# biotite-dev/springcraft

Hardware: AMD Instinct MI355X
Metric: ANM modes/sec (Hessian build + full eigensolve), N=2000 C-alpha (higher is better)
Workload: dtype f64; 1 GPU; C3: N=2000 C-alpha ANM, HinsenForceField (no cutoff), full 6000x6000 eigensolve, all modes + vectors; parallelism=independent structures sharded over GPUs, no data-path collective

## Files before the change

### include/springcraft_hip_debug.h

```cpp
#ifndef SPRINGCRAFT_HIP_DEBUG_H
#define SPRINGCRAFT_HIP_DEBUG_H

#include "springcraft_hip.h"

#ifdef __cplusplus
extern "C" {
#endif

int sc_dbg_gemm_bench(sc_ctx* ctx, int m, int n, int k, int mode, int tile, int split_k, int iters, int beta_one,
                      double* ms_out, double* max_err_out);

int sc_dbg_gemm_host(sc_ctx* ctx, const double* a, const double* b, double* c, int m, int n, int k, int mode, int tile,
                     int split_k, double alpha, double beta, int lower_grid);

int sc_dbg_gemm3_host(sc_ctx* ctx, const double* a, const double* b, double* c, int count, int m, int n, int k, int layout,
                      int lower, double beta);

int sc_dbg_symm3_host(sc_ctx* ctx, const double* a, const double* v, double* x, int count, int m, int split);
int sc_dbg_symm3_stamps(unsigned long long* out4);
int sc_dbg_symm3_bench(sc_ctx* ctx, int count, int m, int split, int iters, double* ms_out);

int sc_dbg_gemm3_bench(sc_ctx* ctx, int count, int m, int n, int k, int layout, int lower, int kernel, int order, int iters,
                       double* ms_out);

int sc_dbg_gemm_stamps(unsigned long long* out4, int reset);

int sc_dbg_gemm_trace(unsigned long long* out, int max_records, int* count, int reset);

int sc_dbg_two_stage(sc_ctx* ctx, const double* a, int n, double* band_out, double* d_out, double* e_out);

int sc_dbg_bt2_stamps(unsigned long long* out);

int sc_dbg_bt2_clock(unsigned long long* out2);

int sc_dbg_bt2_trace(unsigned long long* out);

int sc_dbg_bulge_stamps(unsigned long long* out6);
int sc_dbg_pair_stamps(unsigned long long* out48);
int sc_dbg_chase_stamps(unsigned long long* out16);

int sc_dbg_set_chase(sc_ctx* ctx, int mode, int give_up_after);

int sc_dbg_set_panel_coop(sc_ctx* ctx, int min_rows);
int sc_dbg_set_panel_coop_fail(sc_ctx* ctx, int panel);

int sc_dbg_set_resident(sc_ctx* ctx, int mode, int hook, int workgroups);
int sc_dbg_resident_stamps(unsigned long long* out8);

#ifdef __cplusplus
}
#endif
#endif
```

### springcraft_amd/csrc/api.hip

```cpp
#include <algorithm>
#include <cmath>
#include <cstdarg>
#include <cstring>
#include <map>
#include <new>
#include <utility>

#include "common.h"
#include "host_logic.h"

int sc_set_error(sc_ctx* ctx, int code, const char* fmt, ...) {
  char buf[1024];
  va_list ap;
  va_start(ap, fmt);
  vsnprintf(buf, sizeof(buf), fmt, ap);
  va_end(ap);
  if (ctx) ctx->err = buf;
  return code;
}

static int reserve(sc_ctx* ctx, void*& buf, size_t& have, size_t bytes, bool collect_events = false) {
  if (bytes <= have) return SC_OK;
  if (buf) {
    SC_HIP(ctx, hipStreamSynchronize(ctx->stream));
// ... 98 lines not shown
  SC_HIP(ctx, hipStreamCreateWithFlags(&ctx->aux_stream, hipStreamNonBlocking));
  SC_HIP(ctx, hipEventCreateWithFlags(&ctx->aux_fork, hipEventDisableTiming));
  SC_HIP(ctx, hipEventCreateWithFlags(&ctx->aux_join, hipEventDisableTiming));
  return SC_OK;
}

int sc_side_streams(sc_ctx* ctx, int count) {
  while ((int)ctx->side_streams.size() < count) {
    hipStream_t s = nullptr;
    hipEvent_t e = nullptr;
    SC_HIP(ctx, hipStreamCreateWithFlags(&s, hipStreamNonBlocking));
    if (hipEventCreateWithFlags(&e, hipEventDisableTiming) != hipSuccess) {
      (void)hipStreamDestroy(s);
      return sc_set_error(ctx, SC_ERR_HIP, "hipEventCreateWithFlags failed");
    }
    ctx->side_streams.push_back(s);
    ctx->side_joins.push_back(e);
  }
  return SC_OK;
}

namespace {

int ctx_create_impl(int device, void* stream, bool own, sc_ctx** out) {
  if (!out) return SC_ERR_INVALID_ARG;
  *out = nullptr;
  int count = 0;
  if (hipGetDeviceCount(&count) != hipSuccess || count <= 0 || device < 0 || device >= count)
    return SC_ERR_NO_DEVICE;
  hipDeviceProp_t prop;
  if (hipGetDeviceProperties(&prop, device) != hipSuccess) return SC_ERR_NO_DEVICE;
  if (std::strncmp(prop.gcnArchName, "gfx950", 6) != 0) return SC_ERR_NO_DEVICE;
  if (hipSetDevice(device) != hipSuccess) return SC_ERR_NO_DEVICE;
  sc_ctx* ctx = new sc_ctx();
  ctx->device = device;
  ctx->num_cus = prop.multiProcessorCount;
  if (own) {
    if (hipStreamCreateWithFlags(&ctx->stream, hipStreamNonBlocking) != hipSuccess) {
      delete ctx;
      return SC_ERR_HIP;
    }
    ctx->own_stream = true;
  } else {
    ctx->stream = (hipStream_t)stream;
  }
  if (hipMalloc((void**)&ctx->d_status, kSpStatusWords * sizeof(unsigned long long)) != hipSuccess ||
      hipMemset(ctx->d_status, 0, kSpStatusWords * sizeof(unsigned long long)) != hipSuccess ||
      hipMalloc((void**)&ctx->d_zeros, 16384) != hipSuccess || hipMemset(ctx->d_zeros, 0, 16384) != hipSuccess ||
      hipMalloc((void**)&ctx->d_chase_ctl, kChaseCtlInts * sizeof(int)) != hipSuccess ||
      hipMemset(ctx->d_chase_ctl, 0, kChaseCtlInts * sizeof(int)) != hipSuccess ||
      hipDeviceSynchronize() != hipSuccess) {
    if (ctx->d_status) (void)hipFree(ctx->d_status);
    if (ctx->d_zeros) (void)hipFree(ctx->d_zeros);
    if (ctx->d_chase_ctl) (void)hipFree(ctx->d_chase_ctl);
    if (ctx->own_stream) (void)hipStreamDestroy(ctx->stream);
    delete ctx;
    return SC_ERR_NOMEM;
  }
  *out = ctx;
  return SC_OK;
}

int check_ff(sc_ctx* ctx, const sc_ff_desc* ff) {
  std::string err;
  const int rc = sc_host::check_ff(ff, err);
  return rc == SC_OK ? SC_OK : sc_set_error(ctx, rc, "%s", err.c_str());
}

struct Bump {
  char* base;
  size_t off = 0;
  template <typename T>
  T* take(size_t count) {
    off = align_up(off, 256);
    T* p = reinterpret_cast<T*>(base + off);
    off += count * sizeof(T);
    return p;
  }
};

using sc_host::HostPatch;

int build_patch(sc_ctx* ctx, const sc_patch_desc* pd, int64_t n, HostPatch& hp) {
  std::string err;
  const int rc = sc_host::build_patch(pd, n, hp, err);
  return rc == SC_OK ? SC_OK : sc_set_error(ctx, rc, "%s", err.c_str());
}

int upload_patch(sc_ctx* ctx, const HostPatch& hp, Bump& bump, PatchDev& dev) {
  uint8_t* d_shut = bump.take<uint8_t>(hp.shut.size());
  int32_t* d_rp = bump.take<int32_t>(hp.row_ptr.size());
  int32_t* d_col = bump.take<int32_t>(hp.col.size() + 1);
  int8_t* d_flag = bump.take<int8_t>(hp.flag.size() + 1);
  double* d_gam = bump.take<double>(hp.gam.size() + 1);
  SC_HIP(ctx, hipMemcpyAsync(d_shut, hp.shut.data(), hp.shut.size(), hipMemcpyHostToDevice, ctx->stream));
  SC_HIP(ctx, hipMemcpyAsync(d_rp, hp.row_ptr.data(), hp.row_ptr.size() * 4, hipMemcpyHostToDevice, ctx->stream));
  if (!hp.col.empty()) {
    SC_HIP(ctx, hipMemcpyAsync(d_col, hp.col.data(), hp.col.size() * 4, hipMemcpyHostToDevice, ctx->stream));
    SC_HIP(ctx, hipMemcpyAsync(d_flag, hp.flag.data(), hp.flag.size(), hipMemcpyHostToDevice, ctx->stream));
    SC_HIP(ctx, hipMemcpyAsync(d_gam, hp.gam.data(), hp.gam.size() * 8, hipMemcpyHostToDevice, ctx->stream));
  }
  SC_HIP(ctx, hipStreamSynchronize(ctx->stream));
  dev = PatchDev{d_shut, d_rp, d_col, d_flag, d_gam, hp.mask_gamma};
  return SC_OK;
}

int check_coord_args(sc_ctx* ctx, const double* coord, int64_t n) {
  if (!ctx) return SC_ERR_INVALID_ARG;
  if (n < 0 || n > 2000000) return sc_set_error(ctx, SC_ERR_INVALID_ARG, "bad atom count %lld", (long long)n);
  if (n > 0 && !coord) return sc_set_error(ctx, SC_ERR_INVALID_ARG, "coord is NULL");
  return SC_OK;
}

struct Staged {
  double* d_coord = nullptr;
  double* d_w = nullptr;
  PatchDev patch{};
  bool has_patch = false;
  HostPatch hp;
  sc_tab_desc tab_dev{};
  sc_ff_desc ff_dev{};
};

size_t tab_device_bytes(const sc_ff_desc* ff, int64_t n) {
  if (!ff || ff->kind != SC_FF_TABULATED || !ff->tab) return 0;
  const size_t nb = (size_t)ff->tab->n_bins;
  return align_up(nb * 8, 256) + align_up(3 * 400 * nb * 4, 256) + 2 * align_up((size_t)n * 4, 256) +
         align_up((size_t)n, 256) + 2048;
}

int stage_tab(sc_ctx* ctx, const sc_ff_desc* ff, int64_t n, Staged& st, Bump& bump) {
  st.ff_dev = *ff;
  if (ff->kind != SC_FF_TABULATED) return SC_OK;
  const sc_tab_desc* t = ff->tab;
  const size_t nb = (size_t)t->n_bins;
  for (int64_t i = 0; i < n; ++i)
    if (t->atom_type[i] < 0 || t->atom_type[i] >= 20)
      return sc_set_error(ctx, SC_ERR_INDEX, "amino-acid type %d of atom %lld out of range", t->atom_type[i],
                          (long long)i);
  double* d_edges = bump.take<double>(nb);
  float* d_tab = bump.take<float>(3 * 400 * nb);
  int32_t* d_type = bump.take<int32_t>((size_t)n);
  int32_t* d_chain = bump.take<int32_t>((size_t)n);
  uint8_t* d_bond = bump.take<uint8_t>((size_t)n);
  hipStream_t s = ctx->stream;
  if (t->edges_sq) SC_HIP(ctx, hipMemcpyAsync(d_edges, t->edges_sq, nb * 8, hipMemcpyHostToDevice, s));
  SC_HIP(ctx, hipMemcpyAsync(d_tab, t->bonded, 400 * nb * 4, hipMemcpyHostToDevice, s));
  SC_HIP(ctx, hipMemcpyAsync(d_tab + 400 * nb, t->intra_chain, 400 * nb * 4, hipMemcpyHostToDevice, s));
  SC_HIP(ctx, hipMemcpyAsync(d_tab + 800 * nb, t->inter_chain, 400 * nb * 4, hipMemcpyHostToDevice, s));
  SC_HIP(ctx, hipMemcpyAsync(d_type, t->atom_type, (size_t)n * 4, hipMemcpyHostToDevice, s));
  SC_HIP(ctx, hipMemcpyAsync(d_chain, t->chain, (size_t)n * 4, hipMemcpyHostToDevice, s));
  SC_HIP(ctx, hipMemcpyAsync(d_bond, t->bonded_next, (size_t)n, hipMemcpyHostToDevice, s));
  SC_HIP(ctx, hipStreamSynchronize(s));
  st.tab_dev = *t;
  st.tab_dev.edges_sq = d_edges;
  st.tab_dev.bonded = d_tab;
  st.tab_dev.intra_chain = d_tab + 400 * nb;
  st.tab_dev.inter_chain = d_tab + 800 * nb;
  st.tab_dev.atom_type = d_type;
  st.tab_dev.chain = d_chain;
  st.tab_dev.bonded_next = d_bond;
  st.ff_dev.tab = &st.tab_dev;
  return SC_OK;
}

int stage_inputs(sc_ctx* ctx, const double* coord, int64_t n, const sc_ff_desc* ff, const sc_patch_desc* pd,
                 const double* inv_sqrt_mass, size_t extra_bytes, Staged& st, Bump& bump) {
  SC_TRY(build_patch(ctx, pd, n, st.hp));
  size_t need = align_up((size_t)n * 24, 256) + align_up((size_t)n * 8, 256) + 1024 + extra_bytes +
                tab_device_bytes(ff, n);
  if (st.hp.any) need += st.hp.device_bytes();
  SC_TRY(sc_reserve_scratch(ctx, need));
  bump.base = (char*)ctx->scratch;
  bump.off = 0;
  st.d_coord = bump.take<double>((size_t)n * 3);
  SC_HIP(ctx, hipMemcpyAsync(st.d_coord, coord, (size_t)n * 24, hipMemcpyHostToDevice, ctx->stream));
  if (inv_sqrt_mass) {
    st.d_w = bump.take<double>((size_t)n);
    SC_HIP(ctx, hipMemcpyAsync(st.d_w, inv_sqrt_mass, (size_t)n * 8, hipMemcpyHostToDevice, ctx->stream));
  }
  if (st.hp.any) {
    SC_TRY(upload_patch(ctx, st.hp, bump, st.patch));
    st.has_patch = true;
  }
  SC_TRY(stage_tab(ctx, ff, n, st, bump));
  return SC_OK;
}

}

extern "C" {

int sc_ctx_create(int device, sc_ctx** out) { return ctx_create_impl(device, nullptr, true, out); }

int sc_ctx_create_on_stream(int device, void* hip_stream, sc_ctx** out) {
  return ctx_create_impl(device, hip_stream, false, out);
}

void sc_ctx_destroy(sc_ctx* ctx) {
  if (!ctx) return;
  (void)hipSetDevice(ctx->device);
  (void)hipStreamSynchronize(ctx->stream);
  if (ctx->ws) (void)hipFree(ctx->ws);
  if (ctx->scratch) (void)hipFree(ctx->scratch);
  if (ctx->dc_aux) (void)hipFree(ctx->dc_aux);
  if (ctx->pinv_ws) (void)hipFree(ctx->pinv_ws);
  if (ctx->win_ws) (void)hipFree(ctx->win_ws);
  if (ctx->modes_ws) (void)hipFree(ctx->modes_ws);
  if (ctx->d_status) (void)hipFree(ctx->d_status);
  if (ctx->d_zeros) (void)hipFree(ctx->d_zeros);
  if (ctx->d_chase_ctl) (void)hipFree(ctx->d_chase_ctl);
  for (int c = 0; c < 2; ++c) {
    if (ctx->h_stage[c]) (void)hipHostFree(ctx->h_stage[c]);
    if (ctx->h_stage_done[c]) (void)hipEventDestroy(ctx->h_stage_done[c]);
  }
  if (ctx->aux_stream) {
    (void)hipStreamSynchronize(ctx->aux_stream);
    (void)hipStreamDestroy(ctx->aux_stream);
    (void)hipEventDestroy(ctx->aux_fork);
    (void)hipEventDestroy(ctx->aux_join);
  }
  for (size_t i = 0; i < ctx->side_streams.size(); ++i) {
    (void)hipStreamSynchronize(ctx->side_streams[i]);
    (void)hipStreamDestroy(ctx->side_streams[i]);
    (void)hipEventDestroy(ctx->side_joins[i]);
  }
  if (ctx->own_stream) (void)hipStreamDestroy(ctx->stream);
  delete ctx;
}

const char* sc_last_error(sc_ctx* ctx) { return ctx ? ctx->err.c_str() : "null context"; }

int sc_host_alloc(size_t bytes, void** out) {
  if (!out || bytes == 0) return SC_ERR_INVALID_ARG;
  *out = nullptr;
  void* p = nullptr;
  if (hipHostMalloc(&p, bytes, hipHostMallocDefault) != hipSuccess || !p) {
    (void)hipGetLastError();
    return SC_ERR_NOMEM;
  }
  *out = p;
  return SC_OK;
}

int sc_host_free(void* p) {
  if (!p) return SC_OK;
  return hipHostFree(p) == hipSuccess ? SC_OK : SC_ERR_HIP;
}

int sc_ctx_synchronize(sc_ctx* ctx) {
  if (!ctx) return SC_ERR_INVALID_ARG;
  SC_HIP(ctx, hipSetDevice(ctx->device));
  SC_HIP(ctx, hipStreamSynchronize(ctx->stream));
  return sc_deferred_status(ctx);
}

int sc_device_info(sc_ctx* ctx, char* buf, size_t buflen) {
  if (!ctx || !buf || buflen == 0) return SC_ERR_INVALID_ARG;
  hipDeviceProp_t prop;
  SC_HIP(ctx, hipGetDeviceProperties(&prop, ctx->device));
  snprintf(buf, buflen, "%s %s, %d CUs, %.0f GiB", prop.gcnArchName, prop.name,
           prop.multiProcessorCount, (double)prop.totalGlobalMem / (1 << 30));
  return SC_OK;
}

int sc_ctx_set_profiling(sc_ctx* ctx, int enabled) {
  if (!ctx) return SC_ERR_INVALID_ARG;
  ctx->profiling = enabled != 0;
  return SC_OK;
}

int sc_last_eigh_timings(sc_ctx* ctx, double* out6) {
  if (!ctx || !out6) return SC_ERR_INVALID_ARG;
  for (int i = 0; i < 6; ++i) out6[i] = ctx->last_timings[i];
  return SC_OK;
}

int sc_last_eigh_phase_ms(sc_ctx* ctx, const char* name, double* ms) {
  if (!ctx || !name || !ms) return SC_ERR_INVALID_ARG;
  for (const auto& p : ctx->phases)
    if (p.first == name) { *ms = p.second; return SC_OK; }
  *ms = 0.0;
  return SC_ERR_INVALID_ARG;
}

int sc_ctx_get_counter(sc_ctx* ctx, const char* name, int64_t* value) {
  if (!ctx || !name || !value) return SC_ERR_INVALID_ARG;
  const std::string k(name);
  SC_HIP(ctx, hipSetDevice(ctx->device));
  SC_HIP(ctx, hipStreamSynchronize(ctx->stream));
  SC_TRY(sc_collect_events(ctx));
  int tmin = ctx->chase_tickets[0], tmax = ctx->chase_tickets[0];
  long long tsum = 0;
  for (int x = 0; x < std::max(1, std::min(8, ctx->chase_ctl_xcds)); ++x) {
    tmin = std::min(tmin, ctx->chase_tickets[x]);
    tmax = std::max(tmax, ctx->chase_tickets[x]);
    tsum += ctx->chase_tickets[x];
  }
  if (k == "chase_launches") *value = ctx->cnt_chase_launches;
  else if (k == "chase_pair_launches") *value = ctx->cnt_pair_launches;
  else if (k == "chase_pair_fallbacks") *value = ctx->cnt_pair_fallbacks;
  else if (k == "xcd_count") *value = ctx->nxcd;
  else if (k == "gemm3_launches") *value = ctx->cnt_gemm3_launches;
  else if (k == "symm3_launches") *value = ctx->cnt_symm3_launches;
  else if (k == "resident_launches") *value = ctx->cnt_resident_launches;
  else if (k == "resident_takeovers") *value = ctx->cnt_resident_takeovers;
  else if (k == "resident_rollcall_failures") *value = ctx->cnt_resident_rollcalls;
  else if (k == "resident_lost_waits") *value = ctx->cnt_resident_lost;
  else if (k == "resident_lost_at") *value = ctx->resident_lost_at;
  else if (k == "panel_coop_launches") *value = ctx->cnt_coop_launches;
  else if (k == "panel_coop_timeouts") *value = ctx->cnt_coop_timeouts;
  else if (k == "chase_timeouts") *value = ctx->cnt_chase_timeouts;
  else if (k == "chase_incomplete") *value = ctx->cnt_chase_incomplete;
  else if (k == "chase_resumed") *value = ctx->cnt_chase_resumed;
  else if (k == "chase_sweeps") *value = ctx->cnt_chase_sweeps;
  else if (k == "stepwise_chases") *value = ctx->cnt_stepwise_chases;
  else if (k == "chase_xcd_min") *value = tmin;
  else if (k == "chase_xcd_max") *value = tmax;
  else if (k == "chase_xcd_total") *value = tsum;
  else if (k == "chase_wait_matrix") *value = ctx->chase_wait[0];
  else if (k == "chase_wait_sweep") *value = ctx->chase_wait[1];
  else if (k == "chase_wait_task") *value = ctx->chase_wait[2];
  else { *value = 0; return SC_ERR_INVALID_ARG; }
  return SC_OK;
}

int sc_dbg_set_chase(sc_ctx* ctx, int mode, int give_up_after) {
  if (!ctx || mode < -1 || mode > 5 || give_up_after < 0) return SC_ERR_INVALID_ARG;
  ctx->chase_form = mode == 3 ? 1 : (mode == 4 ? 0 : (mode == 5 ? 2 : -1));
  if (mode > 2) mode = 2;
  ctx->chase_mode = mode;
  ctx->chase_give_up = give_up_after;
  if (mode >= 0) ctx->chase_ok = -1;
  return SC_OK;
}

int sc_dbg_set_panel_coop_fail(sc_ctx* ctx, int panel) {
  if (!ctx || panel < -1) return SC_ERR_INVALID_ARG;
  ctx->coop_fail_panel = panel;
  if (panel >= 0) ctx->coop_ok = -1;
  return SC_OK;
}

int sc_dbg_set_resident(sc_ctx* ctx, int mode, int hook, int workgroups) {
  if (!ctx || mode < -1 || mode > 1 || hook < 0 || workgroups < 0 || workgroups > 256) return SC_ERR_INVALID_ARG;
  ctx->resident_mode = mode;
  ctx->resident_hook = hook;
  ctx->resident_wgs = workgroups;
  if (mode != 0) { ctx->resident_ok = -1; ctx->resident_strikes = 0; }
  return SC_OK;
}

int sc_dbg_set_panel_coop(sc_ctx* ctx, int min_rows) {
  if (!ctx || min_rows < -1 || (min_rows > 0 && min_rows < 128)) return SC_ERR_INVALID_ARG;
  ctx->coop_min_rows = min_rows;
  if (min_rows != 0) ctx->coop_ok = -1;
  return SC_OK;
}

int sc_contacts(sc_ctx* ctx, const double* coord, int64_t n, const sc_ff_desc* ff,
                const sc_patch_desc* patch, int64_t* counts, int64_t* n_pairs) {
  SC_TRY(check_coord_args(ctx, coord, n));
  SC_TRY(check_ff(ctx, ff));
  SC_HIP(ctx, hipSetDevice(ctx->device));
  if (n_pairs) *n_pairs = 0;
  if (n == 0) return SC_OK;
  Staged st;
  Bump bump{};
  SC_TRY(stage_inputs(ctx, coord, n, ff, patch, nullptr, (size_t)n * 8 + 256, st, bump));
  int64_t* d_counts = bump.take<int64_t>((size_t)n);
  SC_TRY(launch_contact_counts(ctx, st.d_coord, n, st.ff_dev, st.has_patch ? &st.patch : nullptr, d_counts));
  std::vector<int64_t> h((size_t)n);
  SC_HIP(ctx, hipMemcpyAsync(h.data(), d_counts, (size_t)n * 8, hipMemcpyDeviceToHost, ctx->stream));
  SC_HIP(ctx, hipStreamSynchronize(ctx->stream));
  int64_t total = 0;
  for (int64_t i = 0; i < n; ++i) total += h[(size_t)i];
  if (counts) std::memcpy(counts, h.data(), (size_t)n * 8);
  if (n_pairs) *n_pairs = total;
  return SC_OK;
}

int sc_pairs(sc_ctx* ctx, const double* coord, int64_t n, const sc_ff_desc* ff,
             const sc_patch_desc* patch, int64_t capacity, int64_t* pairs, double* sq_dist,
             int64_t* n_pairs) {
  SC_TRY(check_coord_args(ctx, coord, n));
  SC_TRY(check_ff(ctx, ff));
  if (capacity < 0 || (capacity > 0 && !pairs))
    return sc_set_error(ctx, SC_ERR_INVALID_ARG, "pairs buffer is NULL");
  SC_HIP(ctx, hipSetDevice(ctx->device));
  if (n_pairs) *n_pairs = 0;
  if (n == 0) return SC_OK;
  Staged st;
  Bump bump{};
  const size_t extra = (size_t)(2 * n + 2) * 8 + (size_t)capacity * 24 + 2048;
  SC_TRY(stage_inputs(ctx, coord, n, ff, patch, nullptr, extra, st, bump));
  int64_t* d_counts = bump.take<int64_t>((size_t)n);
  int64_t* d_off = bump.take<int64_t>((size_t)n + 1);
  int64_t* d_pairs = bump.take<int64_t>((size_t)capacity * 2 + 2);
  double* d_sq = sq_dist ? bump.take<double>((size_t)capacity + 1) : nullptr;
  const PatchDev* pdev = st.has_patch ? &st.patch : nullptr;
  SC_TRY(launch_contact_counts(ctx, st.d_coord, n, st.ff_dev, pdev, d_counts));
  SC_TRY(launch_exclusive_scan_i64(ctx, d_counts, n, d_off));
  int64_t k = 0;
  SC_HIP(ctx, hipMemcpyAsync(&k, d_off + n, 8, hipMemcpyDeviceToHost, ctx->stream));
  SC_HIP(ctx, hipStreamSynchronize(ctx->stream));
  if (n_pairs) *n_pairs = k;
  if (k > capacity)
    return sc_set_error(ctx, SC_ERR_INVALID_ARG, "pair buffer too small: %lld > %lld", (long long)k,
                        (long long)capacity);
  if (k == 0) return SC_OK;
  SC_TRY(launch_pair_fill(ctx, st.d_coord, n, st.ff_dev, pdev, d_off, d_pairs, d_sq));
  SC_HIP(ctx, hipMemcpyAsync(pairs, d_pairs, (size_t)k * 16, hipMemcpyDeviceToHost, ctx->stream));
  if (sq_dist)
    SC_HIP(ctx, hipMemcpyAsync(sq_dist, d_sq, (size_t)k * 8, hipMemcpyDeviceToHost, ctx->stream));
  SC_HIP(ctx, hipStreamSynchronize(ctx->stream));
  return SC_OK;
}

static int assemble_host(sc_ctx* ctx, const double* coord, int64_t n, const sc_ff_desc* ff,
                         const sc_patch_desc* patch, const double* inv_sqrt_mass, double* out,
                         int dim) {
  SC_TRY(check_coord_args(ctx, coord, n));
  SC_TRY(check_ff(ctx, ff));
  if (n > 0 && !out) return sc_set_error(ctx, SC_ERR_INVALID_ARG, "output matrix is NULL");
  SC_HIP(ctx, hipSetDevice(ctx->device));
  if (n == 0) return SC_OK;
  const size_t elems = (size_t)n * n * dim * dim;
  Staged st;
  Bump bump{};
  SC_TRY(stage_inputs(ctx, coord, n, ff, patch, inv_sqrt_mass, elems * 8 + 512, st, bump));
  double* d_m = bump.take<double>(elems);
  const PatchDev* pdev = st.has_patch ? &st.patch : nullptr;
  if (dim == 1)
    SC_TRY(launch_kirchhoff(ctx, st.d_coord, n, 1, st.ff_dev, pdev, st.d_w, d_m, nullptr));
  else
    SC_TRY(launch_hessian(ctx, st.d_coord, n, 1, st.ff_dev, pdev, st.d_w, d_m));
  SC_HIP(ctx, hipMemcpyAsync(out, d_m, elems * 8, hipMemcpyDeviceToHost, ctx->stream));
  SC_HIP(ctx, hipStreamSynchronize(ctx->stream));
  return SC_OK;
}

int sc_kirchhoff_f64(sc_ctx* ctx, const double* coord, int64_t n, const sc_ff_desc* ff,
                     const sc_patch_desc* patch, const double* inv_sqrt_mass, double* kirchhoff) {
  return assemble_host(ctx, coord, n, ff, patch, inv_sqrt_mass, kirchhoff, 1);
}

int sc_hessian_f64(sc_ctx* ctx, const double* coord, int64_t n, const sc_ff_desc* ff,
                   const sc_patch_desc* patch, const double* inv_sqrt_mass, double* hessian) {
  return assemble_host(ctx, coord, n, ff, patch, inv_sqrt_mass, hessian, 3);
}

static int check_pairs(sc_ctx* ctx, int64_t n, const int64_t* pairs, int64_t k, const double* gamma) {
  if (k < 0 || (k > 0 && (!pairs || !gamma)))
    return sc_set_error(ctx, SC_ERR_INVALID_ARG, "pairs / gamma is NULL");
  for (int64_t p = 0; p < 2 * k; ++p)
    if (pairs[p] < 0 || pairs[p] >= n)
      return sc_set_error(ctx, SC_ERR_INDEX, "pair index %lld out of range for %lld atoms",
                          (long long)pairs[p], (long long)n);
  return SC_OK;
}

int sc_kirchhoff_from_pairs_f64(sc_ctx* ctx, int64_t n, const int64_t* pairs, int64_t k,
                                const double* gamma, double* kirchhoff) {
  if (!ctx) return SC_ERR_INVALID_ARG;
  if (n < 0 || (n > 0 && !kirchhoff)) return sc_set_error(ctx, SC_ERR_INVALID_ARG, "bad arguments");
  SC_TRY(check_pairs(ctx, n, pairs, k, gamma));
  SC_HIP(ctx, hipSetDevice(ctx->device));
  if (n == 0) return SC_OK;
  const size_t elems = (size_t)n * n;
  SC_TRY(sc_reserve_scratch(ctx, elems * 8 + (size_t)k * 24 + 4096));
  Bump bump{(char*)ctx->scratch};
  double* d_m = bump.take<double>(elems);
  int64_t* d_pairs = bump.take<int64_t>((size_t)k * 2 + 2);
  double* d_g = bump.take<double>((size_t)k + 1);
  if (k > 0) {
    SC_HIP(ctx, hipMemcpyAsync(d_pairs, pairs, (size_t)k * 16, hipMemcpyHostToDevice, ctx->stream));
    SC_HIP(ctx, hipMemcpyAsync(d_g, gamma, (size_t)k * 8, hipMemcpyHostToDevice, ctx->stream));
  }
  SC_TRY(launch_kirchhoff_from_pairs(ctx, n, d_pairs, k, d_g, d_m));
  SC_HIP(ctx, hipMemcpyAsync(kirchhoff, d_m, elems * 8, hipMemcpyDeviceToHost, ctx->stream));
  SC_HIP(ctx, hipStreamSynchronize(ctx->stream));
  return SC_OK;
}

int sc_hessian_from_pairs_f64(sc_ctx* ctx, const double* coord, int64_t n, const int64_t* pairs,
                              int64_t k, const double* gamma, double* hessian) {
  SC_TRY(check_coord_args(ctx, coord, n));
  if (n > 0 && !hessian) return sc_set_error(ctx, SC_ERR_INVALID_ARG, "output matrix is NULL");
  SC_TRY(check_pairs(ctx, n, pairs, k, gamma));
  SC_HIP(ctx, hipSetDevice(ctx->device));
  if (n == 0) return SC_OK;
  const size_t elems = (size_t)n * n * 9;
  SC_TRY(sc_reserve_scratch(ctx, elems * 8 + (size_t)k * 24 + (size_t)n * 24 + 4096));
  Bump bump{(char*)ctx->scratch};
  double* d_m = bump.take<double>(elems);
  double* d_coord = bump.take<double>((size_t)n * 3);
  int64_t* d_pairs = bump.take<int64_t>((size_t)k * 2 + 2);
  double* d_g = bump.take<double>((size_t)k + 1);
  SC_HIP(ctx, hipMemcpyAsync(d_coord, coord, (size_t)n * 24, hipMemcpyHostToDevice, ctx->stream));
  if (k > 0) {
    SC_HIP(ctx, hipMemcpyAsync(d_pairs, pairs, (size_t)k * 16, hipMemcpyHostToDevice, ctx->stream));
    SC_HIP(ctx, hipMemcpyAsync(d_g, gamma, (size_t)k * 8, hipMemcpyHostToDevice, ctx->stream));
  }
  SC_TRY(launch_hessian_from_pairs(ctx, d_coord, n, d_pairs, k, d_g, d_m));
  SC_HIP(ctx, hipMemcpyAsync(hessian, d_m, elems * 8, hipMemcpyDeviceToHost, ctx->stream));
  SC_HIP(ctx, hipStreamSynchronize(ctx->stream));
  return SC_OK;
}

int sc_eigh_f64(sc_ctx* ctx, const double* a, int64_t n, double* w, double* v) {
  if (!ctx) return SC_ERR_INVALID_ARG;
  if (n < 0 || (n > 0 && (!a || !w))) return sc_set_error(ctx, SC_ERR_INVALID_ARG, "bad arguments");
  SC_HIP(ctx, hipSetDevice(ctx->device));
  if (n == 0) return SC_OK;
  const size_t elems = (size_t)n * n;
  SC_TRY(sc_reserve_scratch(ctx, elems * 8 * (v ? 2 : 1) + (size_t)n * 8 + 4096));
  Bump bump{(char*)ctx->scratch};
  double* d_a = bump.take<double>(elems);
  double* d_w = bump.take<double>((size_t)n);
  double* d_v = v ? bump.take<double>(elems) : nullptr;
  SC_HIP(ctx, hipMemcpyAsync(d_a, a, elems * 8, hipMemcpyHostToDevice, ctx->stream));
  SC_TRY(eigh_batched(ctx, d_a, n, 1, d_w, d_v));
  SC_HIP(ctx, hipMemcpyAsync(w, d_w, (size_t)n * 8, hipMemcpyDeviceToHost, ctx->stream));
  if (v) SC_HIP(ctx, hipMemcpyAsync(v, d_v, elems * 8, hipMemcpyDeviceToHost, ctx->stream));
  SC_HIP(ctx, hipStreamSynchronize(ctx->stream));
  return SC_OK;
}

int sc_pinvh_f64(sc_ctx* ctx, const double* a, int64_t n, double rcond, double* out) {
  if (!ctx) return SC_ERR_INVALID_ARG;
  if (n < 0 || (n > 0 && (!a || !out))) return sc_set_error(ctx, SC_ERR_INVALID_ARG, "bad arguments");
  SC_HIP(ctx, hipSetDevice(ctx->device));
  if (n == 0) return SC_OK;
  const size_t elems = (size_t)n * n;
  SC_TRY(sc_reserve_scratch(ctx, 2 * elems * 8 + 4096));
  Bump bump{(char*)ctx->scratch};
  double* d_a = bump.take<double>(elems);
  double* d_out = bump.take<double>(elems);
  SC_HIP(ctx, hipMemcpyAsync(d_a, a, elems * 8, hipMemcpyHostToDevice, ctx->stream));
  SC_TRY(pinvh_device(ctx, d_a, n, rcond, d_out));
  SC_HIP(ctx, hipMemcpyAsync(out, d_out, elems * 8, hipMemcpyDeviceToHost, ctx->stream));
  SC_HIP(ctx, hipStreamSynchronize(ctx->stream));
  return SC_OK;
}

int sc_eigh_range_f64(sc_ctx* ctx, const double* a, int64_t n, int64_t il, int64_t iu, double* w, double* v) {
  if (!ctx) return SC_ERR_INVALID_ARG;
  if (n <= 0 || !a || !w || il < 0 || iu < il || iu >= n)
    return sc_set_error(ctx, SC_ERR_INVALID_ARG, "bad arguments");
  SC_HIP(ctx, hipSetDevice(ctx->device));
  const int64_t m = iu - il + 1;
  const size_t elems = (size_t)n * n;
  SC_TRY(sc_reserve_scratch(ctx, elems * 8 + (size_t)m * 8 + (v ? (size_t)m * n * 8 : 0) + 4096));
  Bump bump{(char*)ctx->scratch};
  double* d_a = bump.take<double>(elems);
  double* d_w = bump.take<double>((size_t)m);
  double* d_v = v ? bump.take<double>((size_t)m * n) : nullptr;
  SC_HIP(ctx, hipMemcpyAsync(d_a, a, elems * 8, hipMemcpyHostToDevice, ctx->stream));
  SC_TRY(eigh_range_batched(ctx, d_a, n, 1, il, iu, d_w, d_v));
  SC_HIP(ctx, hipMemcpyAsync(w, d_w, (size_t)m * 8, hipMemcpyDeviceToHost, ctx->stream));
  if (v) SC_HIP(ctx, hipMemcpyAsync(v, d_v, (size_t)m * n * 8, hipMemcpyDeviceToHost, ctx->stream));
  SC_HIP(ctx, hipStreamSynchronize(ctx->stream));
  return SC_OK;
}

int sc_anm_eigen_range_f64(sc_ctx* ctx, const double* coord, int64_t n, const sc_ff_desc* ff,
                           const sc_patch_desc* patch, const double* inv_sqrt_mass, int64_t il, int64_t iu,
                           double* w, double* v) {
  SC_TRY(check_coord_args(ctx, coord, n));
  SC_TRY(check_ff(ctx, ff));
  const int64_t dim3n = 3 * n;
  if (n <= 0 || !w || il < 0 || iu < il || iu >= dim3n)
    return sc_set_error(ctx, SC_ERR_INVALID_ARG, "bad arguments");
  SC_HIP(ctx, hipSetDevice(ctx->device));
  const int64_t m = iu - il + 1;
  const size_t elems = (size_t)dim3n * dim3n;
  Staged st;
  Bump bump{};
  SC_TRY(stage_inputs(ctx, coord, n, ff, patch, inv_sqrt_mass,
                      elems * 8 + (size_t)m * 8 + (v ? (size_t)m * dim3n * 8 : 0) + 4096, st, bump));
  double* d_m = bump.take<double>(elems);
  double* d_w = bump.take<double>((size_t)m);
  double* d_v = v ? bump.take<double>((size_t)m * dim3n) : nullptr;
  SC_TRY(launch_hessian(ctx, st.d_coord, n, 1, st.ff_dev, st.has_patch ? &st.patch : nullptr, st.d_w, d_m));
  SC_TRY(eigh_range_batched(ctx, d_m, dim3n, 1, il, iu, d_w, d_v));
  SC_HIP(ctx, hipMemcpyAsync(w, d_w, (size_t)m * 8, hipMemcpyDeviceToHost, ctx->stream));
  if (v) SC_HIP(ctx, hipMemcpyAsync(v, d_v, (size_t)m * dim3n * 8, hipMemcpyDeviceToHost, ctx->stream));
  SC_HIP(ctx, hipStreamSynchronize(ctx->stream));
  return SC_OK;
}

int sc_dev_eigh_range_f64(sc_ctx* ctx, double* d_a, int64_t n, int64_t batch, int64_t il, int64_t iu,
                          double* d_w, double* d_v) {
  if (!ctx) return SC_ERR_INVALID_ARG;
  if (n <= 0 || batch <= 0 || !d_a || !d_w) return sc_set_error(ctx, SC_ERR_INVALID_ARG, "bad arguments");
  SC_HIP(ctx, hipSetDevice(ctx->device));
  return eigh_range_batched_async(ctx, d_a, n, batch, il, iu, d_w, d_v);
}

static int window_results_to_host(sc_ctx* ctx, int64_t m, int64_t n, const double* d_w, const double* d_v, double** w,
                                  double** v) {
  if (m == 0) return SC_OK;
  void* hw = nullptr;
  void* hv = nullptr;
  int rc = sc_host_alloc((size_t)m * 8, &hw);
  if (rc == SC_OK && d_v) rc = sc_host_alloc((size_t)m * n * 8, &hv);
// ... 872 lines not shown
```

### springcraft_amd/csrc/common.h

```cpp
#pragma once

#include <hip/hip_runtime.h>

#include <cstdint>
#include <cstdio>
#include <map>
#include <mutex>
#include <string>
#include <utility>
#include <vector>

#include "../../include/springcraft_hip.h"

struct sc_ctx {
  int device = 0;
  hipStream_t stream = nullptr;
  bool own_stream = false;
  hipStream_t aux_stream = nullptr;
  std::vector<hipStream_t> side_streams;
  std::vector<hipEvent_t> side_joins;
  hipEvent_t aux_fork = nullptr, aux_join = nullptr;
  std::string err;
  int num_cus = 0;

  void* ws = nullptr;
  size_t ws_bytes = 0;
  void* scratch = nullptr;
  size_t scratch_bytes = 0;
  void* dc_aux = nullptr;
  size_t dc_aux_bytes = 0;
  void* pinv_ws = nullptr;
  size_t pinv_ws_bytes = 0;
  void* win_ws = nullptr;
  size_t win_ws_bytes = 0;
  void* modes_ws = nullptr;
  size_t modes_ws_bytes = 0;

  char* h_stage[2] = {nullptr, nullptr};
  size_t h_stage_bytes[2] = {0, 0}, h_stage_off[2] = {0, 0};
  hipEvent_t h_stage_done[2] = {nullptr, nullptr};
  bool h_stage_pending[2] = {false, false};
  int h_stage_cur = 0;
  unsigned long long* d_status = nullptr;

  int two_stage = -1;
  int chase_ok = -1;
  int chase_mode = -1, chase_give_up = 0;
  int chase_form = -1;
  int nxcd = 0;
  int pair_attr = -1;
  long long cnt_pair_fallbacks = 0;
  int gemm3_attr = -1;
  void* d_zeros = nullptr;
  long long cnt_symm3_launches = 0;
  bool gemm3_side_by_side = false;
  long long cnt_gemm3_launches = 0;
  int coop_attr = -1, coop_ok = -1;
  int coop_min_rows = -1;
  int coop_fail_panel = -1;
  int resident_ok = -1, resident_mode = -1, resident_hook = 0, resident_wgs = 0;
  long long cnt_resident_launches = 0, cnt_resident_takeovers = 0, cnt_resident_rollcalls = 0, cnt_resident_lost = 0;
  long long resident_lost_at = -1;
  int resident_strikes = 0;
  int* d_chase_ctl = nullptr;
  int* last_chase_ctl = nullptr;
  int chase_ctl_xcds = 8;
  long long cnt_coop_launches = 0, cnt_coop_timeouts = 0;
  long long cnt_chase_launches = 0, cnt_chase_timeouts = 0, cnt_chase_incomplete = 0, cnt_chase_resumed = 0,
            cnt_chase_sweeps = 0, cnt_stepwise_chases = 0, cnt_pair_launches = 0;
  int chase_tickets[8] = {0, 0, 0, 0, 0, 0, 0, 0};
  int chase_wait[3] = {-1, -1, -1};
  bool profiling = false;
  double last_timings[6] = {0, 0, 0, 0, 0, 0};
  std::vector<std::pair<std::string, double>> phases;
};

class PhaseTimer {
 public:
  PhaseTimer(sc_ctx* ctx, const char* name, hipStream_t st) : ctx_(ctx), name_(name), st_(st), on_(ctx->profiling) {}
  ~PhaseTimer() { for (hipEvent_t e : ev_) (void)hipEventDestroy(e); }
  void start() { mark(); }
  void stop() { mark(); }
  void finish() {
    if (!on_ || ev_.size() < 2) return;
    double total = 0.0;
    if (hipEventSynchronize(ev_.back()) != hipSuccess) return;
    for (size_t i = 0; i + 1 < ev_.size(); i += 2) {
      float ms = 0.f;
      if (hipEventElapsedTime(&ms, ev_[i], ev_[i + 1]) == hipSuccess) total += ms;
    }
    for (auto& p : ctx_->phases)
      if (p.first == name_) { p.second = total; return; }
    ctx_->phases.emplace_back(name_, total);
  }
 private:
  void mark() {
    if (!on_) return;
    hipEvent_t e = nullptr;
    if (hipEventCreate(&e) != hipSuccess) { on_ = false; return; }
    (void)hipEventRecord(e, st_);
    ev_.push_back(e);
  }
  sc_ctx* ctx_;
  std::string name_;
  hipStream_t st_;
  bool on_;
  std::vector<hipEvent_t> ev_;
};

template <int N>
struct ScopedEvents {
  hipEvent_t e[N];
  ScopedEvents() { for (auto& x : e) x = nullptr; }
  ~ScopedEvents() { for (auto& x : e) if (x) (void)hipEventDestroy(x); }
  ScopedEvents(const ScopedEvents&) = delete;
  ScopedEvents& operator=(const ScopedEvents&) = delete;
  hipEvent_t& operator[](int i) { return e[i]; }
  hipEvent_t* begin() { return e; }
  hipEvent_t* end() { return e + N; }
};

int sc_set_error(sc_ctx* ctx, int code, const char* fmt, ...);

#define SC_HIP(ctx, call)                                                              \
  do {                                                                                 \
    hipError_t e__ = (call);                                                           \
    if (e__ != hipSuccess)                                                             \
      return sc_set_error((ctx), e__ == hipErrorOutOfMemory ? SC_ERR_NOMEM : SC_ERR_HIP, \
                          "%s failed: %s (%s:%d)", #call, hipGetErrorString(e__),      \
                          __FILE__, __LINE__);                                         \
  } while (0)

#define SC_TRY(expr)            \
  do {                          \
    int rc__ = (expr);          \
    if (rc__ != SC_OK) return rc__; \
  } while (0)

int sc_reserve_ws(sc_ctx* ctx, size_t bytes);
int sc_reserve_scratch(sc_ctx* ctx, size_t bytes);
int sc_reserve_dc_aux(sc_ctx* ctx, size_t bytes);
int sc_reserve_pinv(sc_ctx* ctx, size_t bytes);
int sc_reserve_win(sc_ctx* ctx, size_t bytes);
int sc_reserve_modes(sc_ctx* ctx, size_t bytes);
int sc_aux_stream(sc_ctx* ctx);
int sc_side_streams(sc_ctx* ctx, int count);
int sc_stage_upload(sc_ctx* ctx, void* d_dst, const void* h_src, size_t bytes);
int sc_stage_end(sc_ctx* ctx);
constexpr int kSpStatusWords = 16;
constexpr int kChaseCtlInts = 32;
int sc_deferred_status(sc_ctx* ctx);
int sc_collect_events(sc_ctx* ctx);

static inline size_t align_up(size_t x, size_t a) { return (x + a - 1) / a * a; }

struct PatchDev {
  const uint8_t* shut;
  const int32_t* row_ptr;
  const int32_t* col;
  const int8_t* flag;
  const double* gam;
  int mask_gamma;
};

int launch_kirchhoff(sc_ctx* ctx, const double* d_coord, int64_t n, int64_t batch,
                     const sc_ff_desc& ff, const PatchDev* patch, const double* d_w,
                     double* d_k, int64_t* d_counts);
int launch_hessian(sc_ctx* ctx, const double* d_coord, int64_t n, int64_t batch,
                   const sc_ff_desc& ff, const PatchDev* patch, const double* d_w, double* d_h);
int launch_contact_counts(sc_ctx* ctx, const double* d_coord, int64_t n, const sc_ff_desc& ff,
                          const PatchDev* patch, int64_t* d_counts);
int launch_pair_fill(sc_ctx* ctx, const double* d_coord, int64_t n, const sc_ff_desc& ff,
                     const PatchDev* patch, const int64_t* d_offsets, int64_t* d_pairs,
                     double* d_sqdist);
int launch_exclusive_scan_i64(sc_ctx* ctx, const int64_t* d_in, int64_t n, int64_t* d_out);
int launch_kirchhoff_from_pairs(sc_ctx* ctx, int64_t n, const int64_t* d_pairs, int64_t k,
                                const double* d_gamma, double* d_k);
int launch_hessian_from_pairs(sc_ctx* ctx, const double* d_coord, int64_t n,
                              const int64_t* d_pairs, int64_t k, const double* d_gamma,
                              double* d_h);
size_t asm_item_bytes();
void asm_item_fill(void* dst, long long atom_off, int n, int ld, const sc_ff_desc& ff_dev, const PatchDev& patch);
int launch_assemble_items(sc_ctx* ctx, int dim, const void* d_items, int64_t count, int max_atoms, bool any_patch,
                          bool any_pad, const double* d_coord, const double* d_w, double* d_matrix,
                          unsigned long long* d_bound_bits);
int launch_items_counts(sc_ctx* ctx, const void* d_items, int64_t count, int max_atoms, bool any_patch,
                        const double* d_coord, int64_t* d_counts);
int launch_items_pair_fill(sc_ctx* ctx, const void* d_items, int64_t count, int max_atoms, bool any_patch,
                           const double* d_coord, const int64_t* d_offsets, int64_t* d_pairs, double* d_sqdist);
int launch_items_from_pairs(sc_ctx* ctx, int dim, const void* d_items, int64_t count, int max_atoms, int64_t order,
                            bool any_pad, const double* d_coord, const int64_t* d_pair_off, int64_t k_total,
                            const int64_t* d_pairs, const double* d_gamma, const double* d_w, double* d_matrix,
                            unsigned long long* d_bound_bits);

struct RaggedRec;

int eigh_batched(sc_ctx* ctx, double* d_a, int64_t n, int64_t batch, double* d_w, double* d_v);
int eigh_batched_async(sc_ctx* ctx, double* d_a, int64_t n, int64_t batch, double* d_w, double* d_v);
size_t eigh_workspace_bytes(int64_t n, int64_t batch, bool want_vectors);
int eigh_range_batched(sc_ctx* ctx, double* d_a, int64_t n, int64_t batch, int64_t il, int64_t iu,
                       double* d_w, double* d_v);
int eigh_range_batched_async(sc_ctx* ctx, double* d_a, int64_t n, int64_t batch, int64_t il, int64_t iu,
                             double* d_w, double* d_v);
int eigh_window_batched_async(sc_ctx* ctx, double* d_a, int64_t n, int64_t batch, double vl, double vu, int64_t K,
                              double* d_w, double* d_v, int64_t* d_count, const RaggedRec* d_own = nullptr);
int eigh_window(sc_ctx* ctx, double* d_a, int64_t n, double vl, double vu, bool vectors, int64_t* m, double** d_w,
                double** d_v);
int pinvh_device(sc_ctx* ctx, double* d_a, int64_t n, double rcond, double* d_out);

size_t modes_scratch_bytes(int64_t n, int dim, int64_t nsel, int what);
int modes_msf_device(sc_ctx* ctx, const double* d_v, const double* d_w, int64_t n, int dim, const int* d_sel,
                     int64_t nsel, char* scratch, double* d_out);
int modes_dcc_device(sc_ctx* ctx, const double* d_v, const double* d_w, int64_t n, int dim, const int* d_sel,
                     int64_t nsel, int norm, char* scratch, double* d_out);
int modes_prs_device(sc_ctx* ctx, const double* d_v, const double* d_w, int64_t n, double rcond, int norm,
                     char* scratch, double* d_out);

struct RaggedRec {
  int own, n_atoms;
  long long atom_off, sq_off;
};
struct RaggedView {
  const RaggedRec* d_rec;
  int first_row, max_atoms;
  int64_t total_atoms, total_sq;
};
size_t modes_budget_default();
int64_t batch_modes_nsel(const sc_mode_selection& sel, int64_t nvec);
size_t batch_modes_workspace_bytes(int64_t m, int64_t nvec, int64_t batch, int dim, int64_t n_sel, int what,
                                   size_t budget, const RaggedView* ragged = nullptr);
int batch_msf_device(sc_ctx* ctx, const double* d_w, const double* d_v, int64_t m, int64_t nvec, int64_t batch, int dim,
                     const sc_mode_selection& sel, const int64_t* d_counts, size_t budget, double* d_out,
                     const RaggedView* ragged = nullptr);
int batch_dcc_device(sc_ctx* ctx, const double* d_w, const double* d_v, int64_t m, int64_t nvec, int64_t batch, int dim,
                     const sc_mode_selection& sel, const int64_t* d_counts, int norm, size_t budget, double* d_out,
                     const RaggedView* ragged = nullptr);
int batch_aniso_device(sc_ctx* ctx, const double* d_w, const double* d_v, int64_t m, int64_t nvec, int64_t batch,
                       const sc_mode_selection& sel, const int64_t* d_counts, size_t budget, double* d_out,
                       const RaggedView* ragged = nullptr);

int modes_overlap_device(sc_ctx* ctx, const double* d_v, int64_t m, int64_t nvec, int64_t batch, int dim,
                         const int* d_rows, int64_t nout, const double* d_disp, int64_t q, const int64_t* d_counts,
                         double* d_overlap, double* d_coll, const RaggedView* ragged = nullptr);

inline bool sc_raise_dyn_lds(const void* fn, int bytes) {
  static std::mutex mu;
  static std::map<std::pair<int, const void*>, bool> done;
  int dev = -1;
  if (hipGetDevice(&dev) != hipSuccess) return false;
  std::lock_guard<std::mutex> g(mu);
  const auto key = std::make_pair(dev, fn);
  const auto it = done.find(key);
  if (it != done.end()) return it->second;
  const bool ok = hipFuncSetAttribute(fn, hipFuncAttributeMaxDynamicSharedMemorySize, bytes) == hipSuccess;
  done[key] = ok;
  return ok;
}
```

### springcraft_amd/csrc/eigh.hip

```cpp
#include <algorithm>
#include <cstdlib>
#include <memory>
#include <vector>

#include "eigh_internal.h"

namespace {

int panel_width() {
  static int nb = [] {
    const char* e = getenv("SPRINGCRAFT_NB");
    const int v = e ? atoi(e) : 64;
    return (v == 128 || v == 96 || v == 64 || v == 32) ? v : 64;
  }();
  return nb;
}
#define kNb (panel_width())

size_t tri_slab_doubles(int n, TriLayout* out) {
  TriLayout L{};
  L.n = n;
  L.nb = kNb;
  const long long nt = (n + 63) / 64 + 1;
  long long off = 0;
  auto take = [&](long long cnt) { long long o = off; off += (cnt + 7) / 8 * 8; return o; };
  L.vw = take((long long)n * 2 * kNb);
  L.wv = take((long long)n * 2 * kNb);
  L.xraw = take(n);
  L.ypart = take(nt * n);
  L.dpart = take(nt * 2 * kNb);
  L.npart = take(nt + 8);
  L.wvpart = take(nt + 8);
  L.d = take(n);
  L.e = take(n);
  L.tau = take(n);
  L.hscale = take(8);
  L.rctl = take(8);
  L.rrec = take(6 * ((n + 63) / 64 * 64));
  L.slab = off;
  if (out) *out = L;
  return (size_t)off;
}

bool two_stage_for(const sc_ctx* ctx, int n, int batch) {
  static const int env_mode = [] {
    const char* e = getenv("SPRINGCRAFT_TWO_STAGE");
    return e ? atoi(e) : -1;
  }();
  const int mode = (ctx && ctx->two_stage >= 0) ? ctx->two_stage : env_mode;
  if (n < 4 * sb_band_width()) return false;
  if (mode == 0) return false;
  if (mode == 1) return true;
  if (batch == 1 && resident_enabled(ctx)) return n > 7000;
  return n >= 512 && (double)batch * n * n >= std::max(1.7e7, 5.0e3 * n);
}

struct Plan {
  TriLayout TL;
  DcLayout DL;
  BtLayout BL;
  SbLayout SL;
  bool two = false;
  size_t off_tri = 0, off_dc = 0, off_bt = 0, off_qtmp = 0, off_u = 0, off_desc = 0, off_sb = 0, off_dia = 0, total = 0;
  int n_syr2k = 0, n_merge = 0, n_bt = 0;
  long long n_bt2 = 0;
};

Plan make_plan(const sc_ctx* ctx, int n, int batch, bool vectors) {
  Plan P;
  size_t off = 0;
  auto take = [&](size_t bytes) { size_t o = off; off += align_up(bytes, 256); return o; };
  P.off_tri = take(tri_slab_doubles(n, &P.TL) * 8 * batch);
  const int npanels = (n + kNb - 1) / kNb;
  P.n_syr2k = npanels * batch;
  P.two = two_stage_for(ctx, n, batch);
  if (P.two) {
    P.off_sb = take(sb_slab_doubles(n, batch, &P.SL) * 8 * batch);
    P.off_dia = take(sizeof(int) * ((size_t)n / 64 + 8));
    P.n_syr2k = std::max(P.n_syr2k, sb_desc_count(n, batch));
  }
  if (vectors) {
    P.off_dc = take(dc_slab_doubles(n, &P.DL) * 8 * batch);
    P.off_bt = take(bt_slab_doubles(n, &P.BL) * 8 * batch);
    P.off_qtmp = take((size_t)n * n * 8 * batch);
    P.off_u = take((size_t)n * n * 8 * batch);
    P.n_merge = 2 * dc_max_nodes(n, P.DL.leaf_max) * batch;
    P.n_bt = bt_desc_count(n, batch);
  }
  P.off_desc = take(sizeof(GemmDesc) * ((size_t)P.n_syr2k + P.n_merge + P.n_bt + (size_t)P.n_bt2 + 8));
  P.total = off;
  return P;
}

__global__ __launch_bounds__(256) void k_sturm(const double* __restrict__ tri_all, TriLayout TL,
                                               double* __restrict__ w_all, long long stride_w) {
  const double* tri = tri_all + (size_t)blockIdx.y * TL.slab;
  const double* d = tri + TL.d;
  const double* e = tri + TL.e;
  const int n = TL.n;
  __shared__ double red[8];
  double lo = 1e300, hi = -1e300, emax = 0.0;
  for (int i = threadIdx.x; i < n; i += blockDim.x) {
    const double el = i > 0 ? fabs(e[i - 1]) : 0.0, er = i < n - 1 ? fabs(e[i]) : 0.0;
    lo = fmin(lo, d[i] - el - er);
    hi = fmax(hi, d[i] + el + er);
    emax = fmax(emax, er);
  }
  for (int off = 32; off > 0; off >>= 1) {
    lo = fmin(lo, __shfl_xor(lo, off));
    hi = fmax(hi, __shfl_xor(hi, off));
    emax = fmax(emax, __shfl_xor(emax, off));
  }
  const int w = threadIdx.x >> 6;
  if ((threadIdx.x & 63) == 0) { red[w] = lo; red[4 + w] = hi; }
  __syncthreads();
  lo = fmin(fmin(red[0], red[1]), fmin(red[2], red[3]));
  hi = fmax(fmax(red[4], red[5]), fmax(red[6], red[7]));
  __syncthreads();
  if ((threadIdx.x & 63) == 0) red[w] = emax;
  __syncthreads();
  emax = fmax(fmax(red[0], red[1]), fmax(red[2], red[3]));
  const double span = fmax(fabs(lo), fabs(hi));
  const double pivmin = fmax(2.2250738585072014e-308 * fmax(1.0, emax * emax), 1e-290);
  lo -= 2.0 * 2.2e-16 * span * n + 2.0 * pivmin;
  hi += 2.0 * 2.2e-16 * span * n + 2.0 * pivmin;

  const int k = blockIdx.x * blockDim.x + threadIdx.x;
  if (k >= n) return;
  if (span == 0.0) {
    w_all[(size_t)blockIdx.y * stride_w + k] = 0.0;
    return;
  }
  double a = lo, b = hi;
  for (int it = 0; it < 120; ++it) {
    const double mid = 0.5 * (a + b);
    if (mid <= a || mid >= b) break;
    int cnt = 0;
    double q = d[0] - mid;
    if (fabs(q) < pivmin) q = -pivmin;
    cnt += q < 0.0;
    for (int i = 1; i < n; ++i) {
      const double ee = e[i - 1];
      q = d[i] - mid - ee * ee / q;
      if (fabs(q) < pivmin) q = -pivmin;
      cnt += q < 0.0;
    }
    if (cnt > k) b = mid; else a = mid;
  }
  w_all[(size_t)blockIdx.y * stride_w + k] = 0.5 * (a + b);
}

}

int sturm_bisect_batched(sc_ctx* ctx, int n, int batch, const double* d_tri_ws, const TriLayout& TL,
                         double* d_w, long long stride_w) {
  hipLaunchKernelGGL(k_sturm, dim3((unsigned)((n + 255) / 256), (unsigned)batch), dim3(256), 0, ctx->stream,
                     d_tri_ws, TL, d_w, stride_w);
  SC_HIP(ctx, hipGetLastError());
  return SC_OK;
}

size_t eigh_workspace_bytes(int64_t n, int64_t batch, bool want_vectors) {
  return make_plan(nullptr, (int)n, (int)batch, want_vectors).total;
}

struct AuxJoinGuard {
  sc_ctx* ctx;
  hipStream_t main;
  bool forked = false, joined = false;
  ~AuxJoinGuard() {
    ctx->stream = main;
    if (forked && !joined) {
      (void)hipEventRecord(ctx->aux_join, ctx->aux_stream);
      (void)hipStreamWaitEvent(main, ctx->aux_join, 0);
    }
  }
};

int eigh_batched_async(sc_ctx* ctx, double* d_a, int64_t n64, int64_t batch64, double* d_w, double* d_v) {
  if (n64 > 46000) return sc_set_error(ctx, SC_ERR_INVALID_ARG, "matrix order %lld too large", (long long)n64);
  const int n = (int)n64, batch = (int)batch64;
  const bool vectors = d_v != nullptr;
  hipStream_t st = ctx->stream;
  const Plan P = make_plan(ctx, n, batch, vectors);
  SC_TRY(sc_reserve_ws(ctx, P.total));
  char* base = (char*)ctx->ws;
  double* tri_ws = (double*)(base + P.off_tri);
  GemmDesc* descs = (GemmDesc*)(base + P.off_desc);
  const long long stride_a = (long long)n * n;

  const int npanels = (n + kNb - 1) / kNb;
  std::vector<GemmDesc> h((size_t)npanels * batch);
  for (int p = 0; p < npanels; ++p) {
    const int pend = std::min((p + 1) * kNb, n);
    for (int b = 0; b < batch; ++b) {
      double* ws = tri_ws + (size_t)b * P.TL.slab;
      GemmDesc D{};
      D.a = ws + P.TL.vw + pend; D.sa_i = 1; D.sa_k = n;
      D.b = ws + P.TL.wv + pend; D.sb_k = n; D.sb_j = 1;
      D.c = d_a + (size_t)b * stride_a + (size_t)pend * n + pend; D.ldc = n;
      D.m = n - pend; D.n = n - pend; D.k = 2 * kNb;
      D.alpha = -1.0; D.beta = 1.0;
      D.lower_only = 1;
      h[(size_t)p * batch + b] = D;
    }
  }
  SC_TRY(sc_stage_upload(ctx, descs, h.data(), h.size() * sizeof(GemmDesc)));

  ScopedEvents<4> ev;
  float ms_bt2 = 0.f;
  const bool prof = ctx->profiling;
  if (prof) {
    for (auto& e : ev) SC_HIP(ctx, hipEventCreate(&e));
    SC_HIP(ctx, hipEventRecord(ev[0], st));
  }
  float ms_symv = 0.f, ms_syr2k = 0.f;
  double* sb_ws = (double*)(base + P.off_sb);
  std::unique_ptr<PhaseTimer> t_tf;
  if (prof) ctx->phases.clear();
  SC_TRY(prepare_matrix_batched(ctx, d_a, stride_a, n, batch, tri_ws, P.TL));
  if (P.two) {
    SC_TRY(sytrd_2stage_batched(ctx, d_a, stride_a, n, batch, tri_ws, P.TL, sb_ws, P.SL, (int*)(base + P.off_dia),
                                descs, &ms_symv, &ms_syr2k));
  } else {
    SC_TRY(tridiag_batched(ctx, d_a, stride_a, n, batch, tri_ws, P.TL, descs, &ms_symv, &ms_syr2k));
  }
  if (prof) SC_HIP(ctx, hipEventRecord(ev[1], st));

  if (!vectors) {
    SC_TRY(sturm_bisect_batched(ctx, n, batch, tri_ws, P.TL, d_w, n));
    SC_TRY(unscale_values_batched(ctx, d_w, n, n, batch, tri_ws, P.TL));
    if (prof) SC_HIP(ctx, hipEventRecord(ev[2], st));
  } else {
    static const bool no_aux = getenv("SPRINGCRAFT_NO_AUX") != nullptr;
    double* dc_ws = (double*)(base + P.off_dc);
    double* bt_ws = (double*)(base + P.off_bt);
    double* q_tmp = (double*)(base + P.off_qtmp);
    double* u = (double*)(base + P.off_u);
    GemmDesc* bt_descs = descs + P.n_syr2k + P.n_merge;
    const int bt_off = P.two ? sb_band_width() : 1;
    static const int aux_single = [] { const char* e = getenv("SPRINGCRAFT_AUX_SINGLE"); return e ? atoi(e) : -1; }();
    const bool single_fork = aux_single >= 0 ? aux_single != 0 : (batch == 1 && resident_enabled(ctx));
    const bool use_aux = !no_aux && (P.two || batch >= 4 || single_fork);
    AuxJoinGuard aux{ctx, st};
    if (P.two && no_aux) {
      t_tf.reset(new PhaseTimer(ctx, "dia_tfactor", st));
      t_tf->start();
      SC_TRY(bt2_prepare(ctx, n, batch, sb_ws, P.SL, st));
      t_tf->stop();
    } else if (use_aux) {
      SC_TRY(backtransform_batched(ctx, d_a, stride_a, n, batch, tri_ws, P.TL, bt_ws, P.BL, d_v, stride_a, n, q_tmp,
                                   bt_descs, bt_off, 1));
      SC_TRY(sc_aux_stream(ctx));
      SC_HIP(ctx, hipEventRecord(ctx->aux_fork, st));
      SC_HIP(ctx, hipStreamWaitEvent(ctx->aux_stream, ctx->aux_fork, 0));
      aux.forked = true;
      if (P.two) {
        t_tf.reset(new PhaseTimer(ctx, "dia_tfactor", ctx->aux_stream));
        t_tf->start();
        SC_TRY(bt2_prepare(ctx, n, batch, sb_ws, P.SL, ctx->aux_stream));
        t_tf->stop();
      }
      {
        ctx->stream = ctx->aux_stream;
        const int rc_prep = backtransform_batched(ctx, d_a, stride_a, n, batch, tri_ws, P.TL, bt_ws, P.BL, d_v, stride_a,
                                                  n, q_tmp, bt_descs, bt_off, 2);
        ctx->stream = st;
        if (rc_prep != SC_OK) return rc_prep;
        SC_HIP(ctx, hipEventRecord(ctx->aux_join, ctx->aux_stream));
      }
    }
    SC_TRY(stedc_batched(ctx, n, batch, tri_ws, P.TL, dc_ws, P.DL, d_w, n, d_v, q_tmp, u, stride_a, descs + P.n_syr2k));
    SC_TRY(unscale_values_batched(ctx, d_w, n, n, batch, tri_ws, P.TL));
    if (prof) SC_HIP(ctx, hipEventRecord(ev[2], st));
    if (use_aux) {
      SC_HIP(ctx, hipStreamWaitEvent(st, ctx->aux_join, 0));
      aux.joined = true;
    }
    if (P.two) SC_TRY(bt2_batched(ctx, n, batch, sb_ws, P.SL, (const int*)(base + P.off_dia), d_v, stride_a, n, &ms_bt2));
    SC_TRY(backtransform_batched(ctx, d_a, stride_a, n, batch, tri_ws, P.TL, bt_ws, P.BL, d_v, stride_a, n, q_tmp,
                                 bt_descs, bt_off, use_aux ? 3 : 0));
  }
  if (prof) {
    SC_HIP(ctx, hipEventRecord(ev[3], st));
    SC_HIP(ctx, hipEventSynchronize(ev[3]));
    float t01 = 0, t12 = 0, t23 = 0;
    SC_HIP(ctx, hipEventElapsedTime(&t01, ev[0], ev[1]));
    SC_HIP(ctx, hipEventElapsedTime(&t12, ev[1], ev[2]));
    SC_HIP(ctx, hipEventElapsedTime(&t23, ev[2], ev[3]));
    ctx->last_timings[0] = t01;
    ctx->last_timings[1] = t12;
    ctx->last_timings[2] = t23;
    ctx->last_timings[3] = ms_symv;
    ctx->last_timings[4] = ms_syr2k;
    ctx->last_timings[5] = 0.0;
    if (P.two) ctx->last_timings[5] = vectors ? ms_bt2 : 1e-9;
    if (t_tf) t_tf->finish();
  }
  return sc_stage_end(ctx);
}

int eigh_batched(sc_ctx* ctx, double* d_a, int64_t n, int64_t batch, double* d_w, double* d_v) {
  SC_TRY(eigh_batched_async(ctx, d_a, n, batch, d_w, d_v));
  SC_HIP(ctx, hipStreamSynchronize(ctx->stream));
  return sc_deferred_status(ctx);
}


namespace {

struct PartialPlan {
  TriLayout TL;
  BtLayout BL;
  SbLayout SL;
  bool two = false, vectors = false;
  int npanels = 0, n_tri_desc = 0;
  size_t off_tri = 0, off_sb = 0, off_dia = 0, off_stein = 0, off_bt = 0, off_vt = 0, off_desc = 0, off_win = 0,
         off_wcopy = 0, total = 0;
};

PartialPlan make_partial_plan(const sc_ctx* ctx, int n, int batch, bool vectors, int m_stein, int window_k) {
  PartialPlan P;
  P.vectors = vectors;
  size_t off = 0;
  auto take = [&](size_t bytes) { size_t o = off; off += align_up(bytes, 256); return o; };
  P.off_tri = take(tri_slab_doubles(n, &P.TL) * 8 * batch);
  P.npanels = (n + kNb - 1) / kNb;
  P.n_tri_desc = P.npanels * batch;
  P.two = two_stage_for(ctx, n, batch);
  int n_bt = 0;
  if (P.two) {
    P.off_sb = take(sb_slab_doubles(n, batch, &P.SL) * 8 * batch);
    P.off_dia = take(sizeof(int) * ((size_t)n / 64 + 8));
    P.n_tri_desc = std::max(P.n_tri_desc, sb_desc_count(n, batch));
  }
  if (vectors) {
    if (m_stein > 0) P.off_stein = take(stein_workspace_doubles(n, m_stein) * 8 * batch);
    P.off_bt = take(bt_slab_doubles(n, &P.BL) * 8 * batch);
    P.off_vt = take((size_t)n * n * 8 * batch);
    n_bt = bt_desc_count(n, batch);
  }
  const size_t n_desc = (size_t)P.n_tri_desc + n_bt + 2 * (size_t)batch + 8;
  P.off_desc = take(sizeof(GemmDesc) * n_desc);
  if (window_k > 0) {
    P.off_win = take(sizeof(WinCount) * batch);
    P.off_wcopy = take(sizeof(double) * batch * (size_t)window_k);
  }
  P.total = off;
  return P;
}

struct PartialProfile {
  sc_ctx* ctx;
  ScopedEvents<4> ev;
  float ms_a = 0.f, ms_b = 0.f, ms_bt2 = 0.f;
  explicit PartialProfile(sc_ctx* c) : ctx(c) {}
  int mark(int i) {
    if (!ctx->profiling) return SC_OK;
    if (i == 0) {
      ctx->phases.clear();
      for (auto& e : ev) SC_HIP(ctx, hipEventCreate(&e));
    }
    SC_HIP(ctx, hipEventRecord(ev[i], ctx->stream));
    return SC_OK;
  }
  int finish(bool two, bool vectors) {
    if (!ctx->profiling) return SC_OK;
    SC_TRY(mark(3));
    SC_HIP(ctx, hipEventSynchronize(ev[3]));
    float t01 = 0, t12 = 0, t23 = 0;
    SC_HIP(ctx, hipEventElapsedTime(&t01, ev[0], ev[1]));
    SC_HIP(ctx, hipEventElapsedTime(&t12, ev[1], ev[2]));
    SC_HIP(ctx, hipEventElapsedTime(&t23, ev[2], ev[3]));
    ctx->last_timings[0] = t01;
    ctx->last_timings[1] = t12;
    ctx->last_timings[2] = t23;
    ctx->last_timings[3] = ms_a;
    ctx->last_timings[4] = ms_b;
    ctx->last_timings[5] = two ? (vectors ? ms_bt2 : 1e-9) : 0.0;
    return SC_OK;
  }
};

int partial_tridiagonalise(sc_ctx* ctx, double* d_a, int n, int batch, const PartialPlan& P, char* base,
                           PartialProfile& prof) {
  const long long stride_a = (long long)n * n;
  double* tri_ws = (double*)(base + P.off_tri);
  GemmDesc* descs = (GemmDesc*)(base + P.off_desc);
// ... 200 lines not shown
```

### springcraft_amd/csrc/eigh_internal.h

```cpp
#pragma once

#include "common.h"
#include "gemm_f64.h"

struct TriLayout {
  int n, nb;
  long long slab;
  long long vw;
  long long wv;
  long long xraw;
  long long ypart;
  long long dpart;
  long long npart;
  long long wvpart;
  long long d, e, tau;
  long long hscale;
  long long rctl;
  long long rrec;
};
inline size_t tri_resident_bytes(int n) { return sizeof(double) * (8 + (size_t)6 * ((n + 63) / 64 * 64)); }

int mirror_lower_batched(sc_ctx* ctx, double* d_a, long long stride_a, int n, int batch);
int prepare_matrix_batched(sc_ctx* ctx, double* d_a, long long stride_a, int n, int batch, double* d_tri_ws,
                           const TriLayout& L);
int unscale_values_batched(sc_ctx* ctx, double* d_w, long long stride_w, int m, int batch, const double* d_tri_ws,
                           const TriLayout& L);

int tridiag_batched(sc_ctx* ctx, double* d_a, long long stride_a, int n, int batch, double* d_ws,
                    const TriLayout& L, const GemmDesc* d_syr2k_descs, float* ms_symv, float* ms_syr2k);
bool resident_enabled(const sc_ctx* ctx);

struct DcNode {
  int lo, mid, hi;
};

struct DcLayout {
  int n;
  int leaf_max;
  long long slab;
  long long dd, ee;
  long long w0, w1;
  long long z;
  long long dl, zz;
  long long ddef;
  long long lam;
  long long tauv;
  long long zhat;
  long long rot_c, rot_s;
  long long scale;
  long long src;
  long long org;
  long long dest;
  long long rot_a, rot_b;
  long long ktop_src, ktop_k;
  long long kbot_src, kbot_k;
  long long cnt;
};

int stedc_batched(sc_ctx* ctx, int n, int batch, const double* d_tri_ws, const TriLayout& TL,
                  double* d_dc_ws, const DcLayout& DL, double* d_w, long long stride_w,
                  double* d_q_out, double* d_q_tmp, double* d_u, long long stride_q,
                  GemmDesc* d_merge_descs );
size_t dc_slab_doubles(int n, DcLayout* out);
int dc_max_nodes(int n, int leaf_max);

int sturm_bisect_batched(sc_ctx* ctx, int n, int batch, const double* d_tri_ws, const TriLayout& TL,
                         double* d_w, long long stride_w);

struct BtLayout {
  int n, nbt, splits;
  long long slab;
  long long vc;
  long long gram;
  long long t;
  long long g12;
  long long tx;
  long long w1;
  long long w2;
  int splits_g;
};
size_t bt_slab_doubles(int n, BtLayout* out);
int bt_desc_count(int n, int batch);
int backtransform_batched(sc_ctx* ctx, double* d_a, long long stride_a, int n, int batch,
                          const double* d_tri_ws, const TriLayout& TL, double* d_bt_ws,
                          const BtLayout& BL, double* d_z, long long stride_z, int ncols, double* d_vt,
                          GemmDesc* d_descs , int off = 1, int phase = 0);

struct SbLayout {
  int n;
  long long slab;
  long long vw, wv;
  long long xv;
  long long qrpart, qrpiv;
  long long qrpart8;
  long long xsplit;
  int symm_split;
  long long small;
  long long cmat;
  long long small2;
  long long p2;
  long long ab;
  int ngroups;
  long long ndia;
  long long vd;
  long long frag;
  long long tau2;
};
size_t sb_slab_doubles(int n, int batch, SbLayout* out);
int sb_desc_count(int n, int batch);
int sb_band_width();
int sytrd_2stage_batched(sc_ctx* ctx, double* d_a, long long stride_a, int n, int batch, double* d_tri_ws,
                         const TriLayout& TL, double* d_sb_ws, const SbLayout& SL, int* d_dia_off ,
                         GemmDesc* d_descs , float* ms_stage1, float* ms_stage2,
                         double* d_band_copy = nullptr);
int bt2_prepare(sc_ctx* ctx, int n, int batch, double* d_sb_ws, const SbLayout& SL, hipStream_t st);
int bt2_batched(sc_ctx* ctx, int n, int batch, double* d_sb_ws, const SbLayout& SL, const int* d_dia_off, double* d_z,
                long long stride_z, int ncols, float* ms_fused = nullptr);

struct WinCount {
  int il, count, start, pad;
};
size_t stein_workspace_doubles(int n, int m);
int stein_batched(sc_ctx* ctx, int n, int batch, const double* d_tri_ws, const TriLayout& TL, int il, int iu,
                  double* d_w, long long stride_w, double* d_x, long long stride_x, double* d_ws,
                  GemmDesc* d_descs , const WinCount* d_win = nullptr);
int window_count_batched(sc_ctx* ctx, int batch, const double* d_tri_ws, const TriLayout& TL, double vl, double vu, int K,
                         WinCount* d_win, long long* d_count, const RaggedRec* d_own = nullptr);
int window_compact_batched(sc_ctx* ctx, int n, int batch, int K, const WinCount* d_win, double* d_w, double* d_v,
                           double* d_w_copy, double* d_v_copy);
```

### springcraft_amd/csrc/gemm3.hip

```cpp
#include <algorithm>
#include <cstdlib>
#include <vector>

#include "gemm_f64.h"

namespace {

typedef double d4 __attribute__((ext_vector_type(4)));
typedef double d2v __attribute__((ext_vector_type(2)));

constexpr int kRow = 1152;
constexpr int kQuarter = 6 * kRow;
constexpr int kSlot = 4 * kQuarter;
constexpr int kRing = 3;
constexpr int kImg = 64 * kRow;
constexpr int kFlagOff = kRing * kSlot + kImg;
constexpr int kG3Lds = kFlagOff + 16;

__device__ __forceinline__ unsigned long long uni64(unsigned long long v) {
  const unsigned lo = (unsigned)__builtin_amdgcn_readfirstlane((int)(unsigned)v);
  const unsigned hi = (unsigned)__builtin_amdgcn_readfirstlane((int)(unsigned)(v >> 32));
  return ((unsigned long long)hi << 32) | lo;
}

struct G3Args {
  const GemmDesc* descs;
  int count, m, n, k;
  int lower;
  int beta_one;
  int order;
  int nwg;
};

template <int LAYOUT>
__global__ __launch_bounds__(1024, 1) void k_gemm3(G3Args P) {
  extern __shared__ __attribute__((aligned(16))) char lds[];
  const int tid = threadIdx.x, lane = tid & 63;
  const int w = __builtin_amdgcn_readfirstlane(tid >> 6);
  const int KS = P.k / 16;
  const int TM = (P.m + 127) >> 7, TN = (P.n + 63) >> 6;
  const int lower = P.lower;
  const int wg = (int)blockIdx.x;
  const int order = P.order;
  const int nwg = P.nwg;
  const int w_first = order == 0 ? wg : (nwg >> 3) * (wg & 7) + (wg >> 3);
  struct It { int z, s, r, tm, tn; bool ok; };
  const int NS = order == 0 ? 1 : (TM + 3) >> 2;
  auto s_rows = [&](int st) { return order == 0 ? TM : min(4, TM - 4 * st); };
  auto s_row0 = [&](int st) { return order == 0 ? 0 : 4 * st; };
  auto s_full = [&](int st) { return lower ? min(TN, 2 * s_row0(st) + 2) : TN; };
  auto s_len = [&](int st) {
    const int h = s_rows(st), r0 = s_row0(st), full = s_full(st);
    int len = h * full;
    if (lower)
      for (int tn = full; tn < TN && (tn >> 1) < r0 + h; ++tn) len += r0 + h - (tn >> 1);
    return len;
  };
  auto it_decode = [&](It& it) {
    const int h = s_rows(it.s), r0 = s_row0(it.s), full = s_full(it.s);
    int r = it.r;
    if (r < h * full) {
      const int c = order == 0 ? r / h : (h == 4 ? r >> 2 : (h == 2 ? r >> 1 : (h == 1 ? r : (r * 43691) >> 17)));
      it.tn = c;
      it.tm = r0 + r - c * h;
      return;
    }
    r -= h * full;
    int tn = full;
    for (;;) {
      const int cnt = r0 + h - (tn >> 1);
      if (r < cnt) break;
      r -= cnt;
      ++tn;
    }
    it.tn = tn;
    it.tm = (tn >> 1) + r;
  };
  auto it_norm = [&](It& it) {
    it.ok = false;
    for (;;) {
      if (it.z >= P.count) return;
      const int len = s_len(it.s);
      if (it.r < len) break;
      it.r -= len;
      if (++it.s == NS) { it.s = 0; ++it.z; }
    }
    it.ok = true;
    it_decode(it);
  };
  auto it_first = [&]() {
    It it;
    it.z = it.s = it.tm = it.tn = 0;
    it.r = w_first;
    it_norm(it);
    return it;
  };
  auto it_next = [&](It& it) {
    if (!it.ok) return;
    it.r += nwg;
    it_norm(it);
  };
  if (!it_first().ok) return;
  const unsigned lds_base = (unsigned)(size_t)(__attribute__((address_space(3))) char*)lds;

  if (w >= 4 && w < 12) {
    const int d = w - 4, q = d & 3, parity = d >> 2;
    It lt = it_first(), cur = lt;
    int l_ks = parity, l_slot = parity % kRing;
    while (lt.ok && l_ks >= KS) { l_ks -= KS; it_next(lt); }
    unsigned long long ab_t = 0, bb_t = 0, lda8 = 0, ldb8 = 0;
    unsigned voff_a[4] = {0, 0, 0, 0}, voff_b0 = 0, voff_b1 = 0;
    bool l_new = true;
    auto issue_group = [&]() {
      if (l_new) {
        const GemmDesc& D = P.descs[lt.z];
        const int row0 = lt.tm * 128, col0 = lt.tn * 64;
        const int mrem = min(128, P.m - row0), nrem = min(64, P.n - col0);
        if (LAYOUT == kGemmAkBk) {
          lda8 = uni64((unsigned long long)D.sa_i * 8ull);
          ab_t = uni64((unsigned long long)(size_t)D.a + (unsigned long long)row0 * lda8);
#pragma unroll
          for (int i = 0; i < 4; ++i)
            voff_a[i] = (unsigned)((unsigned long long)min(32 * q + 8 * i + (lane & 7), mrem - 1) * lda8 + (unsigned)(lane >> 3) * 16u);
        } else {
          lda8 = uni64((unsigned long long)D.sa_k * 8ull);
          ab_t = uni64((unsigned long long)(size_t)D.a + (unsigned long long)row0 * 8ull);
          voff_a[0] = voff_a[1] = voff_a[2] = voff_a[3] = (unsigned)min(lane * 16, (mrem - 2) * 8);
        }
        if (LAYOUT == kGemmAmBn) {
          ldb8 = uni64((unsigned long long)D.sb_k * 8ull);
          bb_t = uni64((unsigned long long)(size_t)D.b + (unsigned long long)col0 * 8ull);
          const int x = (lane >> 4) * 16 + (lane & 7) * 2;
          voff_b0 = voff_b1 = (unsigned)(((lane >> 3) & 1) * (long long)ldb8 + min(x, nrem - 2) * 8);
        } else {
          ldb8 = uni64((unsigned long long)D.sb_j * 8ull);
          bb_t = uni64((unsigned long long)(size_t)D.b + (unsigned long long)col0 * ldb8);
          const int x0 = 16 * q + (lane & 7);
          voff_b0 = (unsigned)((unsigned long long)min(x0, nrem - 1) * ldb8 + (unsigned)(lane >> 3) * 16u);
          voff_b1 = (unsigned)((unsigned long long)min(x0 + 8, nrem - 1) * ldb8 + (unsigned)(lane >> 3) * 16u);
        }
        l_new = false;
      }
      const int k0 = l_ks * 16;
      const int slot_l = l_slot;
      l_ks += 2;
      if (l_ks >= KS) { l_ks -= KS; it_next(lt); l_new = true; }
      l_slot += 2;
      if (l_slot >= kRing) l_slot -= kRing;
      const unsigned m0v = lds_base + (unsigned)(slot_l * kSlot + q * kQuarter + 2880);
      unsigned long long a0, a1, a2, a3, bb0, bb1;
      if (LAYOUT == kGemmAkBk) {
        a0 = a1 = a2 = a3 = ab_t + (unsigned long long)k0 * 8ull;
      } else {
        a0 = ab_t + (unsigned long long)(k0 + 4 * q) * lda8;
        a1 = a0 + lda8; a2 = a1 + lda8; a3 = a2 + lda8;
      }
      if (LAYOUT == kGemmAmBn) {
        bb0 = bb_t + (unsigned long long)(k0 + 4 * q) * ldb8;
        bb1 = bb0 + 2ull * ldb8;
      } else {
        bb0 = bb_t + (unsigned long long)k0 * 8ull;
        bb1 = bb0;
      }
      const unsigned long long s0 = a0 + 2880ull, s1 = a1 + 1728ull, s2 = a2 + 576ull, s3 = a3 - 576ull, s4 = bb0 - 1728ull,
                               s5 = bb1 - 2880ull;
      asm volatile(
          "s_mov_b32 m0, %0\n\ts_nop 4\n\t"
          "global_load_lds_dwordx4 %1, %7 offset:-2880\n\t"
          "global_load_lds_dwordx4 %2, %8 offset:-1728\n\t"
          "global_load_lds_dwordx4 %3, %9 offset:-576\n\t"
          "global_load_lds_dwordx4 %4, %10 offset:576\n\t"
          "global_load_lds_dwordx4 %5, %11 offset:1728\n\t"
          "global_load_lds_dwordx4 %6, %12 offset:2880"
          :
          : "s"(m0v), "v"(voff_a[0]), "v"(voff_a[1]), "v"(voff_a[2]), "v"(voff_a[3]), "v"(voff_b0), "v"(voff_b1), "s"(s0),
            "s"(s1), "s"(s2), "s"(s3), "s"(s4), "s"(s5)
          : "memory");
    };
    if (lt.ok) issue_group();
    asm volatile("s_waitcnt vmcnt(0)" ::: "memory");
    __builtin_amdgcn_s_barrier();
    int c_ks = 0;
    for (int g = 0; cur.ok; ++g) {
      if ((g & 1) == parity) {
        if (lt.ok) issue_group();
      } else {
        asm volatile("s_waitcnt vmcnt(0)" ::: "memory");
      }
      __builtin_amdgcn_s_barrier();
      if (++c_ks == KS) { c_ks = 0; it_next(cur); }
    }
    __builtin_amdgcn_s_barrier();
    return;
  }

  if (w >= 12) {
    const int cw = w - 12;
    const bool with_c = P.beta_one != 0;
    struct CT {
      unsigned long long base, col;
      int row0, colg, mrem, ncol;
      unsigned voff;
    };
    auto ct_of = [&](const It& it) {
      CT t;
      const GemmDesc& D = P.descs[it.z];
      t.row0 = it.tm * 128;
      t.colg = it.tn * 64 + 16 * cw;
      t.mrem = min(128, P.m - t.row0);
      t.ncol = max(0, min(16, P.n - t.colg));
      t.col = uni64((unsigned long long)D.ldc * 8ull);
      t.base = uni64((unsigned long long)(size_t)D.c + (unsigned long long)t.colg * t.col + (unsigned long long)t.row0 * 8ull);
      t.voff = (unsigned)min(lane * 16, (t.mrem - 2) * 8);
      return t;
    };
    auto set_m0 = [&](int h) {
      const unsigned m0v = lds_base + (unsigned)(kRing * kSlot + (16 * cw + 8 * h + 3) * kRow + 576);
      asm volatile("s_mov_b32 m0, %0\n\ts_nop 0" : : "s"(m0v) : "memory");
    };
    auto dma_col = [&](const CT& t, int j) {
      if (j >= t.ncol) return;
      const unsigned long long a = t.base + (unsigned long long)j * t.col;
      switch (j & 7) {
        case 0: { const unsigned long long b = a + 4032ull; asm volatile("s_nop 4\n\tglobal_load_lds_dwordx4 %0, %1 offset:-4032" : : "v"(t.voff), "s"(b) : "memory"); break; }
        case 1: { const unsigned long long b = a + 2880ull; asm volatile("s_nop 4\n\tglobal_load_lds_dwordx4 %0, %1 offset:-2880" : : "v"(t.voff), "s"(b) : "memory"); break; }
        case 2: { const unsigned long long b = a + 1728ull; asm volatile("s_nop 4\n\tglobal_load_lds_dwordx4 %0, %1 offset:-1728" : : "v"(t.voff), "s"(b) : "memory"); break; }
        case 3: { const unsigned long long b = a + 576ull; asm volatile("s_nop 4\n\tglobal_load_lds_dwordx4 %0, %1 offset:-576" : : "v"(t.voff), "s"(b) : "memory"); break; }
        case 4: { const unsigned long long b = a - 576ull; asm volatile("s_nop 4\n\tglobal_load_lds_dwordx4 %0, %1 offset:576" : : "v"(t.voff), "s"(b) : "memory"); break; }
        case 5: { const unsigned long long b = a - 1728ull; asm volatile("s_nop 4\n\tglobal_load_lds_dwordx4 %0, %1 offset:1728" : : "v"(t.voff), "s"(b) : "memory"); break; }
        case 6: { const unsigned long long b = a - 2880ull; asm volatile("s_nop 4\n\tglobal_load_lds_dwordx4 %0, %1 offset:2880" : : "v"(t.voff), "s"(b) : "memory"); break; }
        default: { const unsigned long long b = a - 4032ull; asm volatile("s_nop 4\n\tglobal_load_lds_dwordx4 %0, %1 offset:4032" : : "v"(t.voff), "s"(b) : "memory"); break; }
      }
    };
    const char* img = lds + kRing * kSlot + (16 * cw) * kRow + lane * 16;
    const unsigned voff_st = (unsigned)lane * 16u;
    auto out_col = [&](const CT& t, int j) {
      if (j >= t.ncol) return;
      const int cj = lower == 2 ? ((t.colg + j) & ~1) : t.colg + j;
      const int rel = lower ? max(0, cj - t.row0) : 0;
      if (rel >= t.mrem) return;
      const d2v v = *(const d2v*)(img + j * kRow);
      const unsigned long long a = t.base + (unsigned long long)j * t.col;
      if (rel == 0 && t.mrem == 128) {
        asm volatile("s_nop 4\n\tglobal_store_dwordx4 %0, %1, %2\n\ts_nop 1" : : "v"(voff_st), "v"(v), "s"(a) : "memory");
      } else {
        if (2 * lane >= rel && 2 * lane < t.mrem)
          asm volatile("s_nop 4\n\tglobal_store_dwordx4 %0, %1, %2\n\ts_nop 1" : : "v"(voff_st), "v"(v), "s"(a) : "memory");
        if ((rel & 1) && lane == (rel >> 1)) {
          const double hi = v[1];
          const unsigned long long a8 = a + 8ull;
          asm volatile("s_nop 4\n\tglobal_store_dwordx2 %0, %1, %2\n\ts_nop 1" : : "v"(voff_st), "v"(hi), "s"(a8) : "memory");
        }
      }
    };
    It i_cur = it_first(), i_next = i_cur;
    it_next(i_next);
    CT t_prev{}, t_cur = ct_of(i_cur), t_next{};
    if (i_next.ok) t_next = ct_of(i_next);
    if (with_c) {
      set_m0(0);
      for (int j = 0; j < 8; ++j) dma_col(t_cur, j);
      set_m0(1);
      for (int j = 8; j < 16; ++j) dma_col(t_cur, j);
    }
    asm volatile("s_waitcnt vmcnt(0)" ::: "memory");
    __builtin_amdgcn_s_barrier();
    const int cps = KS >= 13 ? 2 : (KS >= 9 ? 4 : 8);
    const int gsteps = 8 / cps;
    const int first0 = 1, first1 = 1 + gsteps + (KS >= 9 ? 2 : 1);
    for (int t = 0; i_cur.ok; ++t) {
      const bool dma_ok = with_c && i_next.ok;
      const bool st_ok = t > 0;
      for (int ks = 0; ks < KS; ++ks) {
        int j0 = -1;
        if (ks >= first0 && ks < first0 + gsteps) j0 = (ks - first0) * cps;
        if (ks >= first1 && ks < first1 + gsteps) j0 = 8 + (ks - first1) * cps;
        if (j0 >= 0) {
          if (dma_ok && (ks == first0 || ks == first1)) set_m0(j0 >> 3);
          for (int j = j0; j < j0 + cps; ++j) {
            if (st_ok) out_col(t_prev, j);
            if (dma_ok) {
              asm volatile("s_waitcnt lgkmcnt(0)" ::: "memory");
              dma_col(t_next, j);
            }
          }
          asm volatile("s_waitcnt lgkmcnt(0)" ::: "memory");
        }
        if (dma_ok && ks == KS - 1) asm volatile("s_waitcnt vmcnt(0)" ::: "memory");
        if (ks == KS - 1 && cw == 0) {
          *(__attribute__((address_space(3))) int*)(lds + kFlagOff) = i_next.ok ? 1 : 0;
          asm volatile("s_waitcnt lgkmcnt(0)" ::: "memory");
        }
        __builtin_amdgcn_s_barrier();
      }
      t_prev = t_cur;
      t_cur = t_next;
      i_cur = i_next;
      it_next(i_next);
      if (i_next.ok) t_next = ct_of(i_next);
    }
    __builtin_amdgcn_s_barrier();
    for (int j = 0; j < 16; ++j) out_col(t_prev, j);
    return;
  }

  const int wm = w & 1, wn = w >> 1;
  const int fr = lane & 15, fk = lane >> 4;
  __builtin_amdgcn_s_barrier();

  const unsigned a_base = LAYOUT == kGemmAkBk
                              ? (unsigned)((2 * wm) * kQuarter + (fr >> 3) * kRow + (((fk >> 1) * 8 + (fr & 7)) * 16) + (fk & 1) * 8)
                              : (unsigned)(fk * kRow + (wm * 64 + fr) * 8);
  const unsigned b_base = LAYOUT == kGemmAmBn
                              ? (unsigned)(4 * kRow + (fk >> 1) * kRow + (wn * 2) * 256 + (fk & 1) * 128 + fr * 8)
                              : (unsigned)((2 * wn) * kQuarter + 4 * kRow + (fr >> 3) * kRow + (((fk >> 1) * 8 + (fr & 7)) * 16) + (fk & 1) * 8);
  constexpr int kBni = LAYOUT == kGemmAmBn ? 256 : kQuarter, kBk4 = LAYOUT == kGemmAmBn ? kQuarter : 256;
  constexpr int kAk4 = LAYOUT == kGemmAkBk ? 256 : kQuarter;
  auto a_mi = [](int mi) { return LAYOUT == kGemmAkBk ? (mi >> 1) * kQuarter + (mi & 1) * 2 * kRow : mi * 128; };
  char* cimg = lds + kRing * kSlot + (wn * 32 + fk) * kRow + (wm * 64 + fr) * 8;
  const bool with_c = P.beta_one != 0;
  d4 acc[2][4];
#pragma unroll
  for (int ni = 0; ni < 2; ++ni)
#pragma unroll
    for (int r = 0; r < 4; ++r)
#pragma unroll
      for (int mi = 0; mi < 4; ++mi)
        acc[ni][mi][r] = with_c ? *(const double*)(cimg + (ni * 16 + 4 * r) * kRow + mi * 128) : 0.0;

  double af[3][4], bf[3][2];
  auto read_frags = [&](int buf, const char* sp, int k4) {
    const char* pa = sp + a_base;
    const char* pb = sp + b_base;
#pragma unroll
    for (int mi = 0; mi < 4; ++mi) af[buf][mi] = *(const double*)(pa + k4 * kAk4 + a_mi(mi));
#pragma unroll
    for (int ni = 0; ni < 2; ++ni) bf[buf][ni] = *(const double*)(pb + k4 * kBk4 + ni * kBni);
  };
  auto read_frags_asm = [&](int buf, unsigned slot_addr) {
    const unsigned pa = slot_addr + a_base, pb = slot_addr + b_base;
    asm volatile("ds_read_b64 %0, %1" : "=v"(af[buf][0]) : "v"(pa) : "memory");
    if (LAYOUT == kGemmAkBk) {
      asm volatile("ds_read_b64 %0, %1 offset:2304" : "=v"(af[buf][1]) : "v"(pa) : "memory");
      asm volatile("ds_read_b64 %0, %1 offset:6912" : "=v"(af[buf][2]) : "v"(pa) : "memory");
      asm volatile("ds_read_b64 %0, %1 offset:9216" : "=v"(af[buf][3]) : "v"(pa) : "memory");
    } else {
      asm volatile("ds_read_b64 %0, %1 offset:128" : "=v"(af[buf][1]) : "v"(pa) : "memory");
      asm volatile("ds_read_b64 %0, %1 offset:256" : "=v"(af[buf][2]) : "v"(pa) : "memory");
      asm volatile("ds_read_b64 %0, %1 offset:384" : "=v"(af[buf][3]) : "v"(pa) : "memory");
    }
    asm volatile("ds_read_b64 %0, %1" : "=v"(bf[buf][0]) : "v"(pb) : "memory");
    if (LAYOUT == kGemmAmBn) asm volatile("ds_read_b64 %0, %1 offset:256" : "=v"(bf[buf][1]) : "v"(pb) : "memory");
    else asm volatile("ds_read_b64 %0, %1 offset:6912" : "=v"(bf[buf][1]) : "v"(pb) : "memory");
  };
  auto frags_arrived = [&](int buf) {
    asm volatile("s_waitcnt lgkmcnt(0)"
                 : "+v"(af[buf][0]), "+v"(af[buf][1]), "+v"(af[buf][2]), "+v"(af[buf][3]), "+v"(bf[buf][0]), "+v"(bf[buf][1])
                 :
                 : "memory");
  };
  auto mfmas = [&](int buf) {
#pragma unroll
    for (int ni = 0; ni < 2; ++ni)
#pragma unroll
      for (int mi = 0; mi < 4; ++mi)
        acc[ni][mi] = __builtin_amdgcn_mfma_f64_16x16x4f64(bf[buf][ni], af[buf][mi], acc[ni][mi], 0, 0, 0);
  };
  auto swap_all = [&]() {
#pragma unroll
    for (int ni = 0; ni < 2; ++ni)
#pragma unroll
      for (int r2 = 0; r2 < 2; ++r2) {
        double nxt[2][4];
#pragma unroll
        for (int rr = 0; rr < 2; ++rr)
#pragma unroll
          for (int mi = 0; mi < 4; ++mi) nxt[rr][mi] = *(const double*)(cimg + (ni * 16 + 4 * (2 * r2 + rr)) * kRow + mi * 128);
#pragma unroll
        for (int rr = 0; rr < 2; ++rr)
#pragma unroll
          for (int mi = 0; mi < 4; ++mi) {
            *(double*)(cimg + (ni * 16 + 4 * (2 * r2 + rr)) * kRow + mi * 128) = acc[ni][mi][2 * r2 + rr];
            acc[ni][mi][2 * r2 + rr] = with_c ? nxt[rr][mi] : 0.0;
          }
        __builtin_amdgcn_sched_barrier(0);
      }
  };
  read_frags(2, lds, 0);
  read_frags(1, lds, 1);
  mfmas(2);
  int ks = 0, slot = 0;
  bool more = true;
#pragma clang loop unroll(disable)
  while (more) {
    const char* sp = lds + slot * kSlot;
    slot = slot == kRing - 1 ? 0 : slot + 1;
    read_frags(0, sp, 2);
    mfmas(1);
    read_frags(1, sp, 3);
    mfmas(0);
    __builtin_amdgcn_sched_barrier(0);
    asm volatile("s_waitcnt lgkmcnt(0)"
                 :
                 : "v"(af[1][0]), "v"(af[1][1]), "v"(af[1][2]), "v"(af[1][3]), "v"(bf[1][0]), "v"(bf[1][1])
                 : "memory");
    __builtin_amdgcn_s_barrier();
    const char* sn = lds + slot * kSlot;
    const bool boundary = ks == KS - 1;
    ks = boundary ? 0 : ks + 1;
    read_frags_asm(2, lds_base + (unsigned)(slot * kSlot));
    __builtin_amdgcn_sched_barrier(0);
    mfmas(1);
    __builtin_amdgcn_sched_barrier(0);
    frags_arrived(2);
    read_frags(1, sn, 1);
    if (boundary) {
      swap_all();
      more = __builtin_amdgcn_readfirstlane(*(const __attribute__((address_space(3))) int*)(lds + kFlagOff)) != 0;
    }
    mfmas(2);
  }
  asm volatile("s_waitcnt lgkmcnt(0)" ::: "memory");
  __builtin_amdgcn_s_barrier();
}

}

namespace {
bool g_gemm3_any_size = false;
int g_gemm3_order = -1;
}

bool gemm3_would_take(sc_ctx* ctx, int count, int m, int n, int k, int layout, int lower, double alpha, double beta,
                      bool aligned16) {
  static const int env = [] { const char* e = getenv("SPRINGCRAFT_GEMM3"); return e ? atoi(e) : 1; }();
  if (env == 0 || count <= 0) return false;
  if (layout != kGemmAmBn && layout != kGemmAmBk && layout != kGemmAkBk) return false;
  if (alpha != 1.0 || (beta != 0.0 && beta != 1.0)) return false;
  if (!aligned16 || k < 128 || (k & 15) || (m & 1) || m < 2 || n < 1) return false;
  if (layout == kGemmAmBn && (n & 1)) return false;
  if (lower && m != n) return false;
  static const int env_lower = [] { const char* e = getenv("SPRINGCRAFT_GEMM3_LOWER"); return e ? atoi(e) : -1; }();
  if (lower && !g_gemm3_any_size && (env_lower == 0 || (env_lower < 0 && count >= 8 && !ctx->gemm3_side_by_side))) return false;
  if (ctx->num_cus < 256 || ctx->gemm3_attr == 0) return false;
  const long long TM = (m + 127) / 128, TN = (n + 63) / 64;
  const long long hN = TN / 2;
  const long long T1 = lower ? TM * TN - hN * (hN - 1) - ((TN & 1) ? hN : 0) : TM * TN;
  const long long total = T1 * count;
  if (env != 2 && !g_gemm3_any_size && total < 4LL * 256) return false;
  return total <= 0x3fffffffLL;
}

int launch_gemm3_uniform(sc_ctx* ctx, const GemmDesc* d_desc, int count, int m, int n, int k, int layout, int lower,
                         double alpha, double beta, bool aligned16) {
  if (!gemm3_would_take(ctx, count, m, n, k, layout, lower, alpha, beta, aligned16)) return 1;
  if (ctx->gemm3_attr < 0) {
    const bool ok0 = hipFuncSetAttribute(reinterpret_cast<const void*>(&k_gemm3<kGemmAmBk>),
                                         hipFuncAttributeMaxDynamicSharedMemorySize, kG3Lds) == hipSuccess &&
                     hipFuncSetAttribute(reinterpret_cast<const void*>(&k_gemm3<kGemmAkBk>),
                                         hipFuncAttributeMaxDynamicSharedMemorySize, kG3Lds) == hipSuccess;
    const bool ok2 = hipFuncSetAttribute(reinterpret_cast<const void*>(&k_gemm3<kGemmAmBn>),
                                         hipFuncAttributeMaxDynamicSharedMemorySize, kG3Lds) == hipSuccess;
    ctx->gemm3_attr = (ok0 && ok2) ? 1 : 0;
  }
  if (ctx->gemm3_attr != 1) return 1;
  static const int env_order = [] { const char* e = getenv("SPRINGCRAFT_GEMM3_ORDER"); return e ? atoi(e) : 1; }();
  static const int env_lower_wgs = [] { const char* e = getenv("SPRINGCRAFT_GEMM3_LOWER_WGS"); return e ? std::max(8, std::min(256, atoi(e) / 8 * 8)) : 0; }();
  const int nwg = lower ? (env_lower_wgs > 0 ? env_lower_wgs : (ctx->gemm3_side_by_side ? 224 : 256)) : 256;
  G3Args A{d_desc, count, m, n, k, lower, beta != 0.0 ? 1 : 0, g_gemm3_order >= 0 ? g_gemm3_order : env_order, nwg};
  const unsigned grid = (unsigned)nwg;
  if (layout == kGemmAmBn) hipLaunchKernelGGL(k_gemm3<kGemmAmBn>, dim3(grid), dim3(1024), kG3Lds, ctx->stream, A);
  else if (layout == kGemmAkBk) hipLaunchKernelGGL(k_gemm3<kGemmAkBk>, dim3(grid), dim3(1024), kG3Lds, ctx->stream, A);
  else hipLaunchKernelGGL(k_gemm3<kGemmAmBk>, dim3(grid), dim3(1024), kG3Lds, ctx->stream, A);
  if (hipGetLastError() != hipSuccess) {
    ctx->gemm3_attr = 0;
    return 1;
  }
  ++ctx->cnt_gemm3_launches;
  return SC_OK;
}

extern "C" int sc_dbg_gemm3_host(sc_ctx* ctx, const double* a, const double* b, double* c, int count, int m, int n, int k,
                                 int layout, int lower, double beta) {
  if (!ctx || !a || !b || !c || count < 1 || m < 1 || n < 1 || k < 1) return SC_ERR_INVALID_ARG;
  SC_HIP(ctx, hipSetDevice(ctx->device));
  const size_t ea = (size_t)m * k, eb = (size_t)k * n, ec = (size_t)m * n;
  char* base = nullptr;
  SC_HIP(ctx, hipMalloc((void**)&base, (ea + eb + ec) * count * 8 + sizeof(GemmDesc) * (size_t)count + 256));
  double* da = (double*)base;
  double* db = da + ea * count;
  double* dc = db + eb * count;
  GemmDesc* dd = (GemmDesc*)(dc + ec * count);
  int rc = SC_OK;
  auto fail = [&](hipError_t e) { if (e != hipSuccess && rc == SC_OK) rc = sc_set_error(ctx, SC_ERR_HIP, "%s", hipGetErrorString(e)); };
  fail(hipMemcpy(da, a, ea * count * 8, hipMemcpyHostToDevice));
  fail(hipMemcpy(db, b, eb * count * 8, hipMemcpyHostToDevice));
  fail(hipMemcpy(dc, c, ec * count * 8, hipMemcpyHostToDevice));
  std::vector<GemmDesc> h((size_t)count);
  for (int z = 0; z < count; ++z) {
    GemmDesc D{};
    D.a = da + ea * z; D.b = db + eb * z; D.c = dc + ec * z;
    D.m = m; D.n = n; D.k = k; D.ldc = m; D.alpha = 1.0; D.beta = beta;
    D.sa_i = 1; D.sa_k = m;
    if (layout == kGemmAkBk) { D.sa_i = k; D.sa_k = 1; }
    if (layout == kGemmAmBn) { D.sb_k = n; D.sb_j = 1; } else { D.sb_k = 1; D.sb_j = k; }
    D.lower_only = lower;
    h[(size_t)z] = D;
  }
  fail(hipMemcpy(dd, h.data(), sizeof(GemmDesc) * (size_t)count, hipMemcpyHostToDevice));
  if (rc == SC_OK) {
    g_gemm3_any_size = true;
    const int took = launch_gemm3_uniform(ctx, dd, count, m, n, k, layout, lower, 1.0, beta, true);
    g_gemm3_any_size = false;
    if (took != SC_OK) rc = sc_set_error(ctx, SC_ERR_INVALID_ARG, "k_gemm3 does not take m %d n %d k %d layout %d", m, n, k, layout);
    fail(hipStreamSynchronize(ctx->stream));
  }
  if (rc == SC_OK) fail(hipMemcpy(c, dc, ec * count * 8, hipMemcpyDeviceToHost));
  (void)hipFree(base);
  return rc;
}

extern "C" int sc_dbg_gemm3_bench(sc_ctx* ctx, int count, int m, int n, int k, int layout, int lower, int kernel, int order,
                                  int iters, double* ms_out) {
  if (!ctx || count < 1 || iters < 1) return SC_ERR_INVALID_ARG;
  SC_HIP(ctx, hipSetDevice(ctx->device));
  static const int ld_a = [] { const char* e = getenv("SC_DBG_LDA"); return e ? atoi(e) : 0; }();
  static const int ld_c = [] { const char* e = getenv("SC_DBG_LDC"); return e ? atoi(e) : 0; }();
  static const int ld_b = [] { const char* e = getenv("SC_DBG_LDB"); return e ? atoi(e) : 0; }();
  const int lda = std::max(m, ld_a), ldc = std::max(m, ld_c), ldbn = std::max(n, ld_b);
  const size_t ea = (size_t)lda * k, eb = layout == kGemmAmBn ? (size_t)ldbn * k : (size_t)k * n, ec = (size_t)ldc * n;
  char* base = nullptr;
  SC_HIP(ctx, hipMalloc((void**)&base, (ea + eb + ec) * count * 8 + sizeof(GemmDesc) * (size_t)count + 256));
  double* da = (double*)base;
  double* db = da + ea * count;
  double* dc = db + eb * count;
  GemmDesc* dd = (GemmDesc*)(dc + ec * count);
  std::vector<double> hv(std::max(ea, eb));
  unsigned long long sd = 88172645463325252ull;
  for (auto& x : hv) { sd ^= sd << 13; sd ^= sd >> 7; sd ^= sd << 17; x = (double)((long long)(sd % 2001) - 1000) / 1000.0; }
  int rc = SC_OK;
  auto fail = [&](hipError_t e) { if (e != hipSuccess && rc == SC_OK) rc = sc_set_error(ctx, SC_ERR_HIP, "%s", hipGetErrorString(e)); };
  for (int z = 0; z < count; ++z) {
    fail(hipMemcpy(da + ea * z, hv.data(), ea * 8, hipMemcpyHostToDevice));
    fail(hipMemcpy(db + eb * z, hv.data(), eb * 8, hipMemcpyHostToDevice));
  }
  fail(hipMemset(dc, 0, ec * count * 8));
  std::vector<GemmDesc> h((size_t)count);
  for (int z = 0; z < count; ++z) {
    GemmDesc D{};
    D.a = da + ea * z; D.b = db + eb * z; D.c = dc + ec * z;
    D.m = m; D.n = n; D.k = k; D.ldc = ldc; D.alpha = 1.0; D.beta = 1.0;
    D.sa_i = 1; D.sa_k = lda;
    if (layout == kGemmAkBk) { D.sa_i = k; D.sa_k = 1; }
    if (layout == kGemmAmBn) { D.sb_k = ldbn; D.sb_j = 1; } else { D.sb_k = 1; D.sb_j = k; }
    D.lower_only = lower;
    h[(size_t)z] = D;
  }
  fail(hipMemcpy(dd, h.data(), sizeof(GemmDesc) * (size_t)count, hipMemcpyHostToDevice));
  auto launch = [&]() -> int {
    if (kernel == 3) {
      g_gemm3_any_size = true;
      g_gemm3_order = order;
      const int took = launch_gemm3_uniform(ctx, dd, count, m, n, k, layout, lower, 1.0, 1.0, true);
      g_gemm3_any_size = false;
      g_gemm3_order = -1;
      return took == SC_OK ? SC_OK : SC_ERR_INVALID_ARG;
    }
    return launch_gemm_f64(ctx, dd, count, m, n, kGemmTile, 1, false, false, layout, lower != 0 && layout == kGemmAmBn);
  };
  hipEvent_t e0 = nullptr, e1 = nullptr;
  if (rc == SC_OK) {
    fail(hipEventCreate(&e0));
    fail(hipEventCreate(&e1));
    for (int it = 0; it < 2 && rc == SC_OK; ++it) rc = launch();
    fail(hipEventRecord(e0, ctx->stream));
    for (int it = 0; it < iters && rc == SC_OK; ++it) rc = launch();
    fail(hipEventRecord(e1, ctx->stream));
    fail(hipEventSynchronize(e1));
    float ms = 0.f;
    if (rc == SC_OK) fail(hipEventElapsedTime(&ms, e0, e1));
    if (ms_out) *ms_out = ms / iters;
  }
  if (e0) (void)hipEventDestroy(e0);
  if (e1) (void)hipEventDestroy(e1);
  (void)hipFree(base);
  return rc;
}
```

### springcraft_amd/csrc/gemm_f64.h

```cpp
#pragma once

#include <cstdint>

#include "common.h"

struct GemmDesc {
  const double* a;
  const double* b;
  double* c;
  int m, n, k;
  long long sa_i, sa_k;
  long long sb_k, sb_j;
  long long ldc;
  double alpha, beta;
  const int* a_kidx;
  const int* b_kidx;
  const int* c_jidx;
  int lower_only;
  int row_off, col_off;
  long long split_stride;
  int a_tri;
};

constexpr int kGemmTile = 3;

constexpr int kGemmAmBk = 0, kGemmAkBk = 1, kGemmAmBn = 2;
int launch_gemm_f64(sc_ctx* ctx, const GemmDesc* d_desc, int count, int max_m, int max_n, int tile,
                    int split_k = 1, bool gather = false, bool tri = false, int layout = -1, bool lower_grid = false,
                    int pin_tile = 0);
int gemm_f64_tile(const sc_ctx* ctx, int count, int max_m, int max_n, int layout);

int launch_gemm3_uniform(sc_ctx* ctx, const GemmDesc* d_desc, int count, int m, int n, int k, int layout, int lower,
                         double alpha, double beta, bool aligned16);
bool gemm3_would_take(sc_ctx* ctx, int count, int m, int n, int k, int layout, int lower, double alpha, double beta,
                      bool aligned16);

int launch_symm3(sc_ctx* ctx, const GemmDesc* d_desc, int count, int m, int split, bool aligned16, bool any_size = false);
bool symm3_would_take(sc_ctx* ctx, int count, int m, int split, bool aligned16);
```

### springcraft_amd/csrc/stedc.hip

```cpp
#include <algorithm>
#include <vector>

#include "eigh_internal.h"

namespace {

constexpr double kEps = 2.220446049250313e-16;

__device__ __forceinline__ int* iptr(double* ws, long long off) { return reinterpret_cast<int*>(ws + off); }
__device__ __forceinline__ const int* iptr(const double* ws, long long off) {
  return reinterpret_cast<const int*>(ws + off);
}

__device__ __forceinline__ double wave_sum_all(double v) {
#pragma unroll
  for (int off = 32; off > 0; off >>= 1) v += __shfl_xor(v, off);
  return v;
}
__device__ __forceinline__ double wave_prod_all(double v) {
#pragma unroll
  for (int off = 32; off > 0; off >>= 1) v *= __shfl_xor(v, off);
  return v;
}
__device__ __forceinline__ double wave_max_all(double v) {
#pragma unroll
  for (int off = 32; off > 0; off >>= 1) v = fmax(v, __shfl_xor(v, off));
  return v;
}

__global__ void k_dc_prepare(const double* __restrict__ tri_all, TriLayout TL, double* __restrict__ dc_all,
                             DcLayout DL, const DcNode* __restrict__ nodes, int n_nodes) {
  __shared__ double red[16];
  const double* tri = tri_all + (size_t)blockIdx.x * TL.slab;
  double* ws = dc_all + (size_t)blockIdx.x * DL.slab;
  const int n = DL.n, tid = threadIdx.x;
  double mx = 0.0;
  for (int i = tid; i < n; i += blockDim.x) {
    mx = fmax(mx, fabs(tri[TL.d + i]));
    if (i < n - 1) mx = fmax(mx, fabs(tri[TL.e + i]));
  }
  mx = wave_max_all(mx);
  if ((tid & 63) == 0) red[tid >> 6] = mx;
  __syncthreads();
  mx = 0.0;
  for (int w = 0; w < (int)(blockDim.x >> 6); ++w) mx = fmax(mx, red[w]);
  const double nrm = (mx > 0.0 && mx == mx) ? mx : 1.0;
  const double inv = 1.0 / nrm;
  for (int i = tid; i < n; i += blockDim.x) {
    const double dv = tri[TL.d + i] * inv;
    const double ev = (i < n - 1) ? tri[TL.e + i] * inv : 0.0;
    ws[DL.dd + i] = fabs(dv) < 1e-150 ? 0.0 : dv;
    ws[DL.ee + i] = fabs(ev) < 1e-150 ? 0.0 : ev;
  }
  if (tid == 0) ws[DL.scale] = nrm;
  __syncthreads();
  for (int g = tid; g < n_nodes; g += blockDim.x) {
    const int mid = nodes[g].mid;
    const double r = fabs(ws[DL.ee + mid - 1]);
    ws[DL.dd + mid - 1] -= r;
    ws[DL.dd + mid] -= r;
  }
}

template <int LEAF>
__global__ __launch_bounds__(64) void k_dc_leaves(double* __restrict__ dc_all, DcLayout DL,
                                                  const DcNode* __restrict__ leaves,
                                                  double* __restrict__ q_all, long long stride_q,
                                                  int* __restrict__ fail_flag) {
  __shared__ double Z[LEAF][LEAF + 1];
  __shared__ double d[LEAF], e[LEAF];
  double* ws = dc_all + (size_t)blockIdx.y * DL.slab;
  double* Q = q_all + (size_t)blockIdx.y * stride_q;
  const int lo = leaves[blockIdx.x].lo, hi = leaves[blockIdx.x].hi;
  const int s = hi - lo, n = DL.n;
  const int lane = threadIdx.x;
  if (lane < s) {
    for (int c = 0; c < s; ++c) Z[lane][c] = (c == lane) ? 1.0 : 0.0;
    d[lane] = ws[DL.dd + lo + lane];
    e[lane] = (lane < s - 1) ? ws[DL.ee + lo + lane] : 0.0;
  }
  __syncthreads();
  for (int l = 0; l < s; ++l) {
    int iter = 0;
    int m;
    do {
      for (m = l; m < s - 1; ++m) {
        const double dd = fabs(d[m]) + fabs(d[m + 1]);
        if (fabs(e[m]) <= kEps * dd) break;
      }
      if (m != l) {
        if (++iter > 80) {
          if (lane == 0) atomicExch(fail_flag, 1);
          break;
        }
        double g = (d[l + 1] - d[l]) / (2.0 * e[l]);
        double r = hypot(g, 1.0);
        g = d[m] - d[l] + e[l] / (g + copysign(r, g));
        double sn = 1.0, cs = 1.0, p = 0.0;
        int i;
        for (i = m - 1; i >= l; --i) {
          double f = sn * e[i];
          const double b = cs * e[i];
          r = hypot(f, g);
          __syncthreads();
          e[i + 1] = r;
          if (r == 0.0) {
            d[i + 1] -= p;
            e[m] = 0.0;
            __syncthreads();
            break;
          }
          sn = f / r;
          cs = g / r;
          g = d[i + 1] - p;
          r = (d[i] - g) * sn + 2.0 * cs * b;
          p = sn * r;
          d[i + 1] = g + p;
          g = cs * r - b;
          if (lane < s) {
            f = Z[lane][i + 1];
            Z[lane][i + 1] = sn * Z[lane][i] + cs * f;
            Z[lane][i] = cs * Z[lane][i] - sn * f;
          }
          __syncthreads();
        }
        if (r == 0.0 && i >= l) continue;
        __syncthreads();
        d[l] -= p;
        e[l] = g;
        e[m] = 0.0;
        __syncthreads();
      }
    } while (m != l);
  }
  __syncthreads();
  for (int a = 0; a < s - 1; ++a) {
    int k = a;
    double best = d[a];
    for (int b = a + 1; b < s; ++b)
      if (d[b] < best) { best = d[b]; k = b; }
    __syncthreads();
    if (k != a) {
      const double tmp = d[a];
      __syncthreads();
      d[k] = tmp;
      d[a] = best;
      if (lane < s) {
        const double t2 = Z[lane][a];
        Z[lane][a] = Z[lane][k];
        Z[lane][k] = t2;
      }
    }
    __syncthreads();
  }
  if (lane < s) {
    ws[DL.w0 + lo + lane] = d[lane];
    for (int c = 0; c < s; ++c) Q[(size_t)(lo + c) * n + lo + lane] = Z[lane][c];
  }
}

__global__ void k_dc_zero_offdiag(const DcNode* __restrict__ nodes, double* __restrict__ q_all,
                                  long long stride_q, int n) {
  const DcNode nd = nodes[blockIdx.y];
  double* Q = q_all + (size_t)blockIdx.z * stride_q;
  const int n1 = nd.mid - nd.lo, n2 = nd.hi - nd.mid;
  const long long total = 2LL * n1 * n2;
  for (long long idx = blockIdx.x * (long long)blockDim.x + threadIdx.x; idx < total;
       idx += (long long)gridDim.x * blockDim.x) {
    if (idx < (long long)n1 * n2) {
      const int r = nd.mid + (int)(idx % n2), c = nd.lo + (int)(idx / n2);
      Q[(size_t)c * n + r] = 0.0;
    } else {
      const long long k = idx - (long long)n1 * n2;
      const int r = nd.lo + (int)(k % n1), c = nd.mid + (int)(k / n1);
      Q[(size_t)c * n + r] = 0.0;
    }
  }
}

__global__ __launch_bounds__(1024) void k_dc_setup(double* __restrict__ dc_all, DcLayout DL,
                                                   const DcNode* __restrict__ nodes, int nodes_in_level,
                                                   const double* __restrict__ q_all, long long stride_q,
                                                   long long w_old_off, GemmDesc* __restrict__ descs,
                                                   int use_lds, double* __restrict__ gscratch,
                                                   long long gscratch_stride) {
  extern __shared__ __attribute__((aligned(16))) double lds[];
  __shared__ double red[16];
  __shared__ double s_tol;
  const int g = blockIdx.x, b = blockIdx.y;
  const DcNode nd = nodes[g];
  double* ws = dc_all + (size_t)b * DL.slab;
  const double* Q = q_all + (size_t)b * stride_q;
  const int n = DL.n, lo = nd.lo, mid = nd.mid, hi = nd.hi;
  const int N = hi - lo, n1 = mid - lo;
  const int tid = threadIdx.x, nthr = blockDim.x;
  const double* wold = ws + w_old_off;

  double* sd;
  double* sz;
  int* scol;
  unsigned char* smix;
  unsigned char* sflag;
  if (use_lds) {
    sd = lds;
    sz = lds + N;
    scol = reinterpret_cast<int*>(lds + 2 * N);
    smix = reinterpret_cast<unsigned char*>(scol + N);
  } else {
    double* base = gscratch + (size_t)b * gscratch_stride + 3LL * lo;
    sd = base;
    sz = base + N;
    scol = reinterpret_cast<int*>(base + 2 * N);
    smix = reinterpret_cast<unsigned char*>(scol + N);
  }
  sflag = smix + N;

  const double rho_raw = ws[DL.ee + mid - 1];
  const double sgn = rho_raw < 0.0 ? -1.0 : 1.0;
  const double rho = 2.0 * fabs(rho_raw);
  const double isq2 = 0.7071067811865475244;

  double zmax = 0.0, dmax = 0.0;
  for (int j = tid; j < N; j += nthr) {
    const int col = lo + j;
    const double zj = (j < n1 ? Q[(size_t)col * n + (mid - 1)] : sgn * Q[(size_t)col * n + mid]) * isq2;
    ws[DL.z + col] = zj;
    zmax = fmax(zmax, fabs(zj));
    dmax = fmax(dmax, fabs(wold[col]));
  }
  zmax = wave_max_all(zmax);
  dmax = wave_max_all(dmax);
  if ((tid & 63) == 0) red[tid >> 6] = fmax(zmax, dmax);
  __syncthreads();
  if (tid == 0) {
    double mx = 0.0;
    for (int w = 0; w < (nthr >> 6); ++w) mx = fmax(mx, red[w]);
    s_tol = 8.0 * kEps * mx;
  }
  __syncthreads();
  for (int j = tid; j < N; j += nthr) {
    const double v = wold[lo + j];
    int rank;
    if (j < n1) {
      int a = 0, c = N - n1;
      while (a < c) {
        const int h = (a + c) >> 1;
        if (wold[mid + h] < v) a = h + 1; else c = h;
      }
      rank = j + a;
    } else {
      int a = 0, c = n1;
      while (a < c) {
        const int h = (a + c) >> 1;
        if (wold[lo + h] <= v) a = h + 1; else c = h;
      }
      rank = (j - n1) + a;
    }
    sd[rank] = v;
    sz[rank] = ws[DL.z + lo + j];
    scol[rank] = lo + j;
    smix[rank] = 0;
  }
  __syncthreads();

  const double tol = s_tol;
  int* src = iptr(ws, DL.src);
  int* rot_a = iptr(ws, DL.rot_a);
  int* rot_b = iptr(ws, DL.rot_b);
  int* cnt = iptr(ws, DL.cnt);
  int* ktop_src = iptr(ws, DL.ktop_src);
  int* ktop_k = iptr(ws, DL.ktop_k);
  int* kbot_src = iptr(ws, DL.kbot_src);
  int* kbot_k = iptr(ws, DL.kbot_k);
  __shared__ int wsum[3][16];
  __shared__ int s_nrot;
  const int L = (N + nthr - 1) / nthr;
  const int j0 = min(tid * L, N), j1 = min(j0 + L, N);

  for (int j = tid; j < N; j += nthr) sflag[j] = !(rho * fabs(sz[j]) > tol) ? 1 : 0;
  if (tid == 0) s_nrot = 0;
  __syncthreads();
  int nseed = 0;
  for (int jj = j0; jj < j1; ++jj) {
    if (sflag[jj] & 1) continue;
    int pj = jj - 1;
    while (pj >= 0 && (sflag[pj] & 1)) --pj;
    if (pj < 0) continue;
    double s = sz[pj], c = sz[jj];
    const double tau = hypot(c, s);
    const double t = sd[jj] - sd[pj];
    c /= tau;
    s /= tau;
    if (fabs(t * c * s) <= tol) { sflag[jj] |= 2; ++nseed; }
  }
  const int any_rot = __syncthreads_or(nseed);
  if (any_rot) {
    int is = nseed;
    for (int off = 1; off < 64; off <<= 1) {
      const int us = __shfl_up(is, off);
      if ((tid & 63) >= off) is += us;
    }
    if ((tid & 63) == 63) wsum[0][tid >> 6] = is;
    __syncthreads();
    int bs = 0, total = 0;
    for (int w = 0; w < (nthr >> 6); ++w) {
      if (w < (tid >> 6)) bs += wsum[0][w];
      total += wsum[0][w];
    }
    int pos = bs + is - nseed;
    for (int jj = j0; jj < j1; ++jj)
      if (sflag[jj] & 2) kbot_k[lo + pos++] = jj;
    __syncthreads();
    if (tid == 0) {
      int nrot = 0, done_upto = -1;
      for (int si = 0; si < total; ++si) {
        int jj = kbot_k[lo + si];
        if (jj <= done_upto) continue;
        int pj = jj - 1;
        while (pj >= 0 && (sflag[pj] & 5)) --pj;
        while (true) {
          double s = sz[pj], c = sz[jj];
          const double tau = hypot(c, s);
          const double t = sd[jj] - sd[pj];
          c /= tau;
          s /= tau;
          done_upto = jj;
          if (!(fabs(t * c * s) <= tol)) break;
          sz[jj] = tau;
          sz[pj] = 0.0;
          rot_a[lo + nrot] = scol[pj];
          rot_b[lo + nrot] = scol[jj];
          ws[DL.rot_c + lo + nrot] = c;
          ws[DL.rot_s + lo + nrot] = s;
          ++nrot;
          if (((scol[pj] < mid) != (scol[jj] < mid)) || smix[pj] || smix[jj]) { smix[jj] = 1; smix[pj] = 1; }
          const double tt = sd[pj] * c * c + sd[jj] * s * s;
          sd[jj] = sd[pj] * s * s + sd[jj] * c * c;
          sd[pj] = tt;
          sflag[pj] |= 4;
          pj = jj;
          ++jj;
          while (jj < N && (sflag[jj] & 1)) ++jj;
          if (jj >= N) break;
        }
      }
      s_nrot = nrot;
    }
    __syncthreads();
  }
  {
    int ns = 0, nt = 0, nb = 0;
    for (int j = j0; j < j1; ++j)
      if (!(sflag[j] & 5)) {
        const bool top = scol[j] < mid;
        ++ns;
        nt += (top || smix[j]) ? 1 : 0;
        nb += (!top || smix[j]) ? 1 : 0;
      }
    int is = ns, it = nt, ib = nb;
    for (int off = 1; off < 64; off <<= 1) {
      const int us = __shfl_up(is, off), ut = __shfl_up(it, off), ub = __shfl_up(ib, off);
      if ((tid & 63) >= off) { is += us; it += ut; ib += ub; }
    }
    __syncthreads();
    if ((tid & 63) == 63) { wsum[0][tid >> 6] = is; wsum[1][tid >> 6] = it; wsum[2][tid >> 6] = ib; }
    __syncthreads();
    int bs = 0, bt = 0, bb = 0, ts = 0, tt = 0, tb = 0;
    for (int w = 0; w < (nthr >> 6); ++w) {
      if (w < (tid >> 6)) { bs += wsum[0][w]; bt += wsum[1][w]; bb += wsum[2][w]; }
      ts += wsum[0][w];
      tt += wsum[1][w];
      tb += wsum[2][w];
    }
    int K = bs + is - ns, K1 = bt + it - nt, K3 = bb + ib - nb;
    int ndef = j0 - K;
    for (int j = j0; j < j1; ++j) {
      if (sflag[j] & 5) {
        ws[DL.ddef + hi - 1 - ndef] = sd[j];
        src[hi - 1 - ndef] = scol[j];
        ++ndef;
      } else {
        ws[DL.dl + lo + K] = sd[j];
        ws[DL.zz + lo + K] = sz[j];
        src[lo + K] = scol[j];
        const bool top = scol[j] < mid;
        if (top || smix[j]) { ktop_src[lo + K1] = scol[j]; ktop_k[lo + K1] = K; ++K1; }
        if (!top || smix[j]) { kbot_src[lo + K3] = scol[j]; kbot_k[lo + K3] = K; ++K3; }
        ++K;
      }
    }
    if (tid == 0) {
      cnt[2 * g] = ts;
      cnt[2 * g + 1] = s_nrot;
      GemmDesc& Dt = descs[((size_t)b * nodes_in_level + g) * 2];
      Dt.n = ts;
      Dt.k = tt;
      GemmDesc& Db = descs[((size_t)b * nodes_in_level + g) * 2 + 1];
      Db.n = ts;
      Db.k = tb;
    }
  }
}

__global__ void k_dc_rotate(double* __restrict__ dc_all, DcLayout DL, const DcNode* __restrict__ nodes,
                            double* __restrict__ q_all, long long stride_q) {
  const int g = blockIdx.y, b = blockIdx.z;
  const DcNode nd = nodes[g];
  double* ws = dc_all + (size_t)b * DL.slab;
  const int nrot = iptr(ws, DL.cnt)[2 * g + 1];
  if (nrot == 0) return;
  double* Q = q_all + (size_t)b * stride_q;
  const int n = DL.n;
  const int row = nd.lo + blockIdx.x * blockDim.x + threadIdx.x;
  if (row >= nd.hi) return;
  const int* rot_a = iptr(ws, DL.rot_a) + nd.lo;
  const int* rot_b = iptr(ws, DL.rot_b) + nd.lo;
  for (int q = 0; q < nrot; ++q) {
    const double c = ws[DL.rot_c + nd.lo + q], s = ws[DL.rot_s + nd.lo + q];
    double* pa = Q + (size_t)rot_a[q] * n + row;
    double* pb = Q + (size_t)rot_b[q] * n + row;
    const double qa = *pa, qb = *pb;
    *pa = c * qa - s * qb;
    *pb = s * qa + c * qb;
  }
}

__global__ __launch_bounds__(1024) void k_dc_secular(double* __restrict__ dc_all, DcLayout DL,
                                                     const DcNode* __restrict__ nodes, int use_lds) {
  extern __shared__ __attribute__((aligned(16))) double lds[];
  const int g = blockIdx.y, b = blockIdx.z;
  const DcNode nd = nodes[g];
  double* ws = dc_all + (size_t)b * DL.slab;
  const int K = iptr(ws, DL.cnt)[2 * g];
  const int waves = blockDim.x >> 6;
  if ((int)blockIdx.x * waves >= K) return;
  const int lo = nd.lo;
  const double* dlg = ws + DL.dl + lo;
  const double* zzg = ws + DL.zz + lo;
  const double* dl;
  const double* z2;
  if (use_lds) {
    double* ldl = lds;
    double* lz2 = lds + K;
    for (int i = threadIdx.x; i < K; i += blockDim.x) {
      ldl[i] = dlg[i];
      const double z = zzg[i];
      lz2[i] = z * z;
    }
    __syncthreads();
    dl = ldl;
    z2 = lz2;
  } else {
    dl = dlg;
    z2 = nullptr;
  }
  const int lane = threadIdx.x & 63;
  const int j = blockIdx.x * waves + (threadIdx.x >> 6);
  if (j >= K) return;
  const double rho = 2.0 * fabs(ws[DL.ee + nd.mid - 1]);
  const double rinv = 1.0 / rho;

  auto fsum2 = [&](double dorg, double tau, double& fp) -> double {
    double s = 0.0, sp = 0.0;
    if (z2) {
      for (int i = lane; i < K; i += 64) {
        const double r = 1.0 / ((dl[i] - dorg) - tau);
        const double zr = z2[i] * r;
        s += zr;
        sp += zr * r;
      }
    } else {
      for (int i = lane; i < K; i += 64) {
        const double z = zzg[i];
        const double r = 1.0 / ((dl[i] - dorg) - tau);
        const double zr = z * z * r;
        s += zr;
        sp += zr * r;
      }
    }
    fp = wave_sum_all(sp);
    return rinv + wave_sum_all(s);
  };
  auto fsum = [&](double dorg, double tau) -> double {
    double fp;
    return fsum2(dorg, tau, fp);
  };

  int org;
  bool positive;
  double t_hi;
  double t_start = 0.0;
  double zj2 = 0.0, zk2 = 0.0;
  if (j == K - 1) {
    org = K - 1;
    positive = true;
    double s2 = 0.0;
    if (z2) { for (int i = lane; i < K; i += 64) s2 += z2[i]; }
    else { for (int i = lane; i < K; i += 64) s2 += zzg[i] * zzg[i]; }
    s2 = wave_sum_all(s2);
    t_hi = rho * s2 * (1.0 + 8.0 * kEps) + 1e-300;
  } else {
    const double gap = dl[j + 1] - dl[j];
    const double half = 0.5 * gap;
    const double fm = fsum(dl[j], half);
    if (fm > 0.0) { org = j; positive = true; } else { org = j + 1; positive = false; }
    t_hi = half;
    {
      zj2 = z2 ? z2[j] : zzg[j] * zzg[j];
      zk2 = z2 ? z2[j + 1] : zzg[j + 1] * zzg[j + 1];
      const double c = fm + (zj2 - zk2) / half;
      double t0;
      if (positive) {
        const double a = c * gap + zj2 + zk2, b = zj2 * gap;
        const double disc = sqrt(fabs(a * a - 4.0 * b * c));
        t0 = a > 0.0 ? 2.0 * b / (a + disc) : (a - disc) / (2.0 * c);
      } else {
        const double a = c * gap - zj2 - zk2, b = zk2 * gap;
        const double disc = sqrt(fabs(a * a + 4.0 * b * c));
        t0 = -(a < 0.0 ? 2.0 * b / (a - disc) : -(a + disc) / (2.0 * c));
      }
      if (t0 == t0 && t0 > 0.0 && t0 < t_hi) t_start = t0;
    }
  }
  const double dorg = dl[org];
  unsigned long long lo_b = 0ull, hi_b = (unsigned long long)__double_as_longlong(t_hi);
  unsigned long long t_b = hi_b - ((hi_b - lo_b) >> 1);
  if (t_start > 0.0) t_b = (unsigned long long)__double_as_longlong(t_start);
  unsigned long long probe_dist = 4ull;
  double t_accept = 0.0;
  for (int it = 0; it < 90 && hi_b - lo_b > 1ull; ++it) {
    const double t = __longlong_as_double((long long)t_b);
    double fp;
    const double f = fsum2(dorg, positive ? t : -t, fp);
    const bool go_up = positive ? (f < 0.0) : (f > 0.0);
    if (go_up) lo_b = t_b; else hi_b = t_b;
    if (hi_b - lo_b <= 1ull) break;
    const unsigned long long mid_b = lo_b + ((hi_b - lo_b) >> 1);
    double tn;
    bool model_step = false;
    if (j < K - 1 && fabs(f) * t < 0.25 * (positive ? zj2 : zk2)) {
      model_step = true;
      const double tau = positive ? t : -t;
      const double dj = (dl[j] - dorg) - tau, dk = (dl[j + 1] - dorg) - tau;
      const double dw = fp;
      double c;
      if (positive) {
        const double q = zj2 / (dj * dj);
        c = f - dk * dw - (dl[j] - dl[j + 1]) * q;
      } else {
        const double q = zk2 / (dk * dk);
        c = f - dj * dw - (dl[j + 1] - dl[j]) * q;
      }
      const double a = (dj + dk) * f - dj * dk * dw;
      const double b = dj * dk * f;
      double eta;
      if (c == 0.0) {
        eta = a != 0.0 ? b / a : -f / dw;
      } else {
        const double disc = sqrt(fabs(a * a - 4.0 * b * c));
        eta = a <= 0.0 ? (a - disc) / (2.0 * c) : 2.0 * b / (a + disc);
      }
      if (f * eta >= 0.0) eta = -f / dw;
      const double tau_n = tau + eta;
      tn = positive ? tau_n : -tau_n;
    } else {
      const double fpt = positive ? fp : -fp;
      const double den = fpt * t + f;
      tn = fpt * t * t / den;
    }
    unsigned long long n_b = mid_b;
    if (tn == tn && tn > 0.0 && tn < 1.7e308) {
      const unsigned long long c_b = (unsigned long long)__double_as_longlong(tn);
      if (c_b > lo_b && c_b < hi_b) {
        n_b = c_b;
        const unsigned long long step = c_b > t_b ? c_b - t_b : t_b - c_b;
#ifndef DC_STRICT_BRACKET
        if (step <= 2ull || (model_step && fabs(tn - t) <= 1e-12 * t)) {
          t_accept = tn;
          break;
        }
#endif
        if (step <= 4ull) {
          const unsigned long long far = go_up ? c_b + probe_dist : (c_b > probe_dist ? c_b - probe_dist : 0ull);
          n_b = (far > lo_b && far < hi_b) ? far : mid_b;
          probe_dist *= 8ull;
        }
      }
    }
    t_b = n_b;
  }
  double t_best = __longlong_as_double((long long)hi_b);
  if (t_accept > 0.0) {
    t_best = t_accept;
  } else if (lo_b > 0ull) {
    const double t_lo = __longlong_as_double((long long)lo_b);
    const double f_lo = fabs(fsum(dorg, positive ? t_lo : -t_lo));
    const double f_hi = fabs(fsum(dorg, positive ? t_best : -t_best));
    if (f_lo < f_hi) t_best = t_lo;
  }
  if (lane == 0) {
    const double tau = positive ? t_best : -t_best;
    iptr(ws, DL.org)[lo + j] = org;
    ws[DL.tauv + lo + j] = tau;
    ws[DL.lam + lo + j] = dorg + tau;
  }
}

__global__ __launch_bounds__(256) void k_dc_zhat(double* __restrict__ dc_all, DcLayout DL,
                                                 const DcNode* __restrict__ nodes) {
  const int g = blockIdx.y, b = blockIdx.z;
  const DcNode nd = nodes[g];
  double* ws = dc_all + (size_t)b * DL.slab;
  const int K = iptr(ws, DL.cnt)[2 * g];
  const int i = blockIdx.x * (blockDim.x >> 6) + (threadIdx.x >> 6);
  if (i >= K) return;
  const int lane = threadIdx.x & 63, lo = nd.lo;
  const double* dl = ws + DL.dl + lo;
  const int* org = iptr(ws, DL.org) + lo;
  const double* tauv = ws + DL.tauv + lo;
  const double di = dl[i];
  double prod = 1.0;
  for (int j = lane; j < K; j += 64) {
    const double num = (di - dl[org[j]]) - tauv[j];
    prod *= (j == i) ? num : num / (di - dl[j]);
  }
  prod = wave_prod_all(prod);
  if (lane == 0) ws[DL.zhat + lo + i] = copysign(sqrt(fabs(prod)), ws[DL.zz + lo + i]);
}

__global__ __launch_bounds__(256) void k_dc_vectors(double* __restrict__ dc_all, DcLayout DL,
                                                    const DcNode* __restrict__ nodes,
                                                    double* __restrict__ u_all, long long stride_u) {
  __shared__ double red[4];
  const int g = blockIdx.y, b = blockIdx.z;
  const DcNode nd = nodes[g];
  double* ws = dc_all + (size_t)b * DL.slab;
  const int K = iptr(ws, DL.cnt)[2 * g];
  const int j = blockIdx.x;
  if (j >= K) return;
  const int lo = nd.lo, n = DL.n;
  const double* dl = ws + DL.dl + lo;
  const double* zh = ws + DL.zhat + lo;
  const double dorg = dl[iptr(ws, DL.org)[lo + j]];
  const double tau = ws[DL.tauv + lo + j];
  double* U = u_all + (size_t)b * stride_u + (size_t)(lo + j) * n + lo;
  double ss = 0.0;
  for (int i = threadIdx.x; i < K; i += blockDim.x) {
    const double u = zh[i] / ((dl[i] - dorg) - tau);
    U[i] = u;
    ss += u * u;
  }
  ss = wave_sum_all(ss);
  if ((threadIdx.x & 63) == 0) red[threadIdx.x >> 6] = ss;
  __syncthreads();
  const double inv = 1.0 / sqrt((red[0] + red[1]) + (red[2] + red[3]));
  for (int i = threadIdx.x; i < K; i += blockDim.x) U[i] *= inv;
}

__global__ __launch_bounds__(256) void k_dc_finalize(double* __restrict__ dc_all, DcLayout DL,
                                                     const DcNode* __restrict__ nodes, long long w_new_off) {
  const int g = blockIdx.y, b = blockIdx.z;
  const DcNode nd = nodes[g];
  double* ws = dc_all + (size_t)b * DL.slab;
  const int K = iptr(ws, DL.cnt)[2 * g];
  const int lo = nd.lo, hi = nd.hi, N = hi - lo, ndef = N - K;
  const int idx = blockIdx.x * blockDim.x + threadIdx.x;
  if (idx >= N) return;
  const double* lam = ws + DL.lam + lo;
  int* dest = iptr(ws, DL.dest);
  double* wnew = ws + w_new_off;
  auto defval = [&](int e) { return ws[DL.ddef + hi - 1 - e]; };
  if (idx < K) {
    const double v = lam[idx];
    int c = 0;
    for (int e = 0; e < ndef; ++e) c += defval(e) < v;
    dest[lo + idx] = lo + idx + c;
    wnew[lo + idx + c] = v;
  } else {
    const int e = idx - K;
    const double v = defval(e);
    int a = 0, c = K;
    while (a < c) {
      const int h = (a + c) >> 1;
      if (lam[h] <= v) a = h + 1; else c = h;
    }
    int r = a;
    for (int f = 0; f < ndef; ++f) {
      const double u = defval(f);
      r += (u < v) || (u == v && f < e);
    }
    dest[lo + idx] = lo + r;
    wnew[lo + r] = v;
  }
}

__global__ __launch_bounds__(256) void k_dc_copy_deflated(double* __restrict__ dc_all, DcLayout DL,
                                                          const DcNode* __restrict__ nodes,
                                                          const double* __restrict__ q_old_all,
                                                          double* __restrict__ q_new_all,
                                                          long long stride_q) {
  const int g = blockIdx.y, b = blockIdx.z;
  const DcNode nd = nodes[g];
  double* ws = dc_all + (size_t)b * DL.slab;
  const int K = iptr(ws, DL.cnt)[2 * g];
  const int lo = nd.lo, hi = nd.hi, N = hi - lo;
  const int e = blockIdx.x;
  if (e >= N - K) return;
  const int n = DL.n;
  const int scol = iptr(ws, DL.src)[hi - 1 - e];
  const int dcol = iptr(ws, DL.dest)[lo + K + e];
  const double* qs = q_old_all + (size_t)b * stride_q + (size_t)scol * n + lo;
  double* qd = q_new_all + (size_t)b * stride_q + (size_t)dcol * n + lo;
  for (int r = threadIdx.x; r < N; r += blockDim.x) qd[r] = qs[r];
}

__global__ void k_dc_unscale(const double* __restrict__ dc_all, DcLayout DL, long long w_off,
                             double* __restrict__ w_out, long long stride_w) {
  const double* ws = dc_all + (size_t)blockIdx.y * DL.slab;
  const int i = blockIdx.x * blockDim.x + threadIdx.x;
  if (i < DL.n) w_out[(size_t)blockIdx.y * stride_w + i] = ws[w_off + i] * ws[DL.scale];
}

struct Tree {
  std::vector<DcNode> leaves;
  std::vector<std::vector<DcNode>> levels;
};

Tree build_tree(int n, int leaf_max) {
  int depth = 0;
  while (((n + (1 << depth) - 1) >> depth) > leaf_max) ++depth;
  std::vector<std::vector<DcNode>> by_depth(depth + 1);
  by_depth[0].push_back(DcNode{0, n / 2, n});
  for (int dlev = 0; dlev < depth; ++dlev) {
    for (const DcNode& nd : by_depth[dlev]) {
      by_depth[dlev + 1].push_back(DcNode{nd.lo, nd.lo + (nd.mid - nd.lo) / 2, nd.mid});
      by_depth[dlev + 1].push_back(DcNode{nd.mid, nd.mid + (nd.hi - nd.mid) / 2, nd.hi});
    }
  }
  Tree t;
  t.leaves = by_depth[depth];
  for (int dlev = depth - 1; dlev >= 0; --dlev) t.levels.push_back(by_depth[dlev]);
  return t;
}

constexpr int kLeafMax = 32;
constexpr int kLdsCapSetup = 7000;
constexpr int kLdsCapSecular = 9800;

}

int dc_max_nodes(int n, int leaf_max) {
  Tree t = build_tree(n, leaf_max);
  size_t total = t.leaves.size();
  for (auto& l : t.levels) total += l.size();
  return (int)total;
}

size_t dc_slab_doubles(int n, DcLayout* out) {
  DcLayout L{};
  L.n = n;
  L.leaf_max = kLeafMax;
  long long off = 0;
  const long long nn = ((long long)n + 7) / 8 * 8;
  auto take = [&](long long cnt) { long long o = off; off += (cnt + 7) / 8 * 8; return o; };
  L.dd = take(nn); L.ee = take(nn); L.w0 = take(nn); L.w1 = take(nn); L.z = take(nn);
  L.dl = take(nn); L.zz = take(nn); L.ddef = take(nn); L.lam = take(nn); L.tauv = take(nn);
  L.zhat = take(nn); L.rot_c = take(nn); L.rot_s = take(nn); L.scale = take(8);
  L.src = take(nn); L.org = take(nn); L.dest = take(nn); L.rot_a = take(nn); L.rot_b = take(nn);
  L.ktop_src = take(nn); L.ktop_k = take(nn); L.kbot_src = take(nn); L.kbot_k = take(nn);
  L.cnt = take(2LL * dc_max_nodes(n, kLeafMax) + 8);
  L.slab = off;
  if (out) *out = L;
  return (size_t)off;
}

__global__ __launch_bounds__(1024) void k_dc_desc_flops(const GemmDesc* __restrict__ d, int count, double* __restrict__ out) {
  __shared__ double part[16];
  double a = 0.0;
  for (int r = threadIdx.x; r < count; r += 1024) a += 2.0 * (double)d[r].m * (double)d[r].n * (double)d[r].k;
#pragma unroll
  for (int off = 32; off > 0; off >>= 1) a += __shfl_xor(a, off);
  if ((threadIdx.x & 63) == 0) part[threadIdx.x >> 6] = a;
  __syncthreads();
  if (threadIdx.x == 0) {
    double t = 0.0;
    for (int w = 0; w < 16; ++w) t += part[w];
    *out = t;
  }
}

int stedc_batched(sc_ctx* ctx, int n, int batch, const double* d_tri_ws, const TriLayout& TL,
                  double* d_dc_ws, const DcLayout& DL, double* d_w, long long stride_w, double* d_q_out,
                  double* d_q_tmp, double* d_u, long long stride_q, GemmDesc* d_merge_descs) {
  hipStream_t st = ctx->stream;
  Tree tree = build_tree(n, kLeafMax);
  const int nlev = (int)tree.levels.size();

  std::vector<DcNode> flat(tree.leaves);
  std::vector<size_t> lev_off(nlev);
  for (int l = 0; l < nlev; ++l) {
    lev_off[l] = flat.size();
    flat.insert(flat.end(), tree.levels[l].begin(), tree.levels[l].end());
  }
  const size_t n_internal = flat.size() - tree.leaves.size();
  const size_t node_bytes = align_up(flat.size() * sizeof(DcNode), 256);
  const size_t big_bytes = n > kLdsCapSetup ? (size_t)batch * 3 * n * sizeof(double) : 0;
  SC_TRY(sc_reserve_dc_aux(ctx, node_bytes + 256 + big_bytes));
  DcNode* d_nodes = reinterpret_cast<DcNode*>(ctx->dc_aux);
  int* d_fail = reinterpret_cast<int*>(ctx->d_status + 1);
  double* d_big = big_bytes ? reinterpret_cast<double*>(reinterpret_cast<char*>(d_nodes) + node_bytes + 256) : nullptr;
  SC_TRY(sc_stage_upload(ctx, d_nodes, flat.data(), flat.size() * sizeof(DcNode)));

  auto qbuf = [&](int stage) { return ((nlev - stage) % 2 == 0) ? d_q_out : d_q_tmp; };

  std::vector<GemmDesc> h_descs;
  std::vector<size_t> desc_off(nlev);
  for (int l = 0; l < nlev; ++l) {
    desc_off[l] = h_descs.size();
    const auto& nodes = tree.levels[l];
    const double* q_old = qbuf(l);
    double* q_new = qbuf(l + 1);
    for (int b = 0; b < batch; ++b)
      for (size_t g = 0; g < nodes.size(); ++g) {
        const DcNode& nd = nodes[g];
        auto ip = [&](long long off) { return reinterpret_cast<const int*>(d_dc_ws + (size_t)b * DL.slab + off) + nd.lo; };
        for (int half = 0; half < 2; ++half) {
          const int r0 = half == 0 ? nd.lo : nd.mid;
          GemmDesc D{};
          D.a = q_old + (size_t)b * stride_q + r0;
          D.sa_i = 1; D.sa_k = n;
          D.a_kidx = ip(half == 0 ? DL.ktop_src : DL.kbot_src);
          D.b = d_u + (size_t)b * stride_q + (size_t)nd.lo * n + nd.lo;
          D.sb_k = 1; D.sb_j = n;
          D.b_kidx = ip(half == 0 ? DL.ktop_k : DL.kbot_k);
          D.c = q_new + (size_t)b * stride_q + r0;
          D.ldc = n;
          D.c_jidx = ip(DL.dest);
          D.m = half == 0 ? nd.mid - nd.lo : nd.hi - nd.mid; D.n = 0; D.k = 0;
          D.alpha = 1.0; D.beta = 0.0;
          h_descs.push_back(D);
        }
      }
  }
  if (!h_descs.empty()) SC_TRY(sc_stage_upload(ctx, d_merge_descs, h_descs.data(), h_descs.size() * sizeof(GemmDesc)));

  hipLaunchKernelGGL(k_dc_prepare, dim3((unsigned)batch), dim3(1024), 0, st, d_tri_ws, TL, d_dc_ws, DL,
                     d_nodes + tree.leaves.size(), (int)n_internal);
  hipLaunchKernelGGL((k_dc_leaves<kLeafMax>), dim3((unsigned)tree.leaves.size(), (unsigned)batch), dim3(64),
                     0, st, d_dc_ws, DL, d_nodes, qbuf(0), stride_q, d_fail);

  PhaseTimer t_gemm(ctx, "dc_gemm", st);
  for (int l = 0; l < nlev; ++l) {
    const auto& nodes = tree.levels[l];
    const int G = (int)nodes.size();
    const DcNode* dn = d_nodes + lev_off[l];
    int maxN = 0;
    for (auto& nd : nodes) maxN = std::max(maxN, nd.hi - nd.lo);
    double* q_old = qbuf(l);
    double* q_new = qbuf(l + 1);
    const long long w_old = (l % 2 == 0) ? DL.w0 : DL.w1;
    const long long w_new = (l % 2 == 0) ? DL.w1 : DL.w0;
    GemmDesc* descs = d_merge_descs + desc_off[l];

    hipLaunchKernelGGL(k_dc_zero_offdiag,
                       dim3((unsigned)std::min(1024, (maxN * maxN / 2 + 255) / 256 + 1), (unsigned)G,
                            (unsigned)batch),
                       dim3(256), 0, st, dn, q_old, stride_q, n);
    {
      const int use_lds = maxN <= kLdsCapSetup ? 1 : 0;
      const size_t lds = use_lds ? (size_t)maxN * 22 + 32 : 0;
      const int threads = maxN >= 1024 ? 1024 : (maxN >= 256 ? 256 : 64);
      hipLaunchKernelGGL(k_dc_setup, dim3((unsigned)G, (unsigned)batch), dim3(threads), lds, st, d_dc_ws, DL,
                         dn, G, q_old, stride_q, w_old, descs, use_lds, d_big, (long long)3 * n);
    }
    hipLaunchKernelGGL(k_dc_rotate, dim3((unsigned)((maxN + 255) / 256), (unsigned)G, (unsigned)batch),
                       dim3(256), 0, st, d_dc_ws, DL, dn, q_old, stride_q);
    {
      const int use_lds = maxN <= kLdsCapSecular ? 1 : 0;
      const int threads = maxN >= 2048 ? 1024 : 256;
      const int waves = threads / 64;
      const size_t lds = use_lds ? (size_t)maxN * 16 + 16 : 0;
      hipLaunchKernelGGL(k_dc_secular, dim3((unsigned)((maxN + waves - 1) / waves), (unsigned)G, (unsigned)batch),
                         dim3(threads), lds, st, d_dc_ws, DL, dn, use_lds);
    }
    hipLaunchKernelGGL(k_dc_zhat, dim3((unsigned)((maxN + 3) / 4), (unsigned)G, (unsigned)batch), dim3(256), 0,
                       st, d_dc_ws, DL, dn);
    hipLaunchKernelGGL(k_dc_vectors, dim3((unsigned)maxN, (unsigned)G, (unsigned)batch), dim3(256), 0, st,
                       d_dc_ws, DL, dn, d_u, stride_q);
    hipLaunchKernelGGL(k_dc_finalize, dim3((unsigned)((maxN + 255) / 256), (unsigned)G, (unsigned)batch),
                       dim3(256), 0, st, d_dc_ws, DL, dn, w_new);
    hipLaunchKernelGGL(k_dc_copy_deflated, dim3((unsigned)maxN, (unsigned)G, (unsigned)batch), dim3(256), 0, st,
                       d_dc_ws, DL, dn, q_old, q_new, stride_q);
    t_gemm.start();
    SC_TRY(launch_gemm_f64(ctx, descs, 2 * G * batch, (maxN + 1) / 2, maxN, kGemmTile, 1, true, false,
                           kGemmAmBk));
    t_gemm.stop();
  }
  const long long w_final = (nlev % 2 == 0) ? DL.w0 : DL.w1;
  hipLaunchKernelGGL(k_dc_unscale, dim3((unsigned)((n + 255) / 256), (unsigned)batch), dim3(256), 0, st,
                     d_dc_ws, DL, w_final, d_w, stride_w);
  SC_HIP(ctx, hipGetLastError());

  t_gemm.finish();
  if (ctx->profiling && !h_descs.empty()) {
    double* d_flops = reinterpret_cast<double*>(reinterpret_cast<char*>(d_nodes) + node_bytes);
    hipLaunchKernelGGL(k_dc_desc_flops, dim3(1), dim3(1024), 0, st, d_merge_descs, (int)h_descs.size(), d_flops);
    double h_flops = 0.0;
    SC_HIP(ctx, hipMemcpyAsync(&h_flops, d_flops, sizeof(double), hipMemcpyDeviceToHost, st));
    SC_HIP(ctx, hipStreamSynchronize(st));
    bool found = false;
    for (auto& ph : ctx->phases)
      if (ph.first == "dc_gemm_gflop") { ph.second = h_flops * 1e-9; found = true; }
    if (!found) ctx->phases.emplace_back("dc_gemm_gflop", h_flops * 1e-9);
  }
  return SC_OK;
}
```

Measured before the change: 179,100 modes/s.

## Route divide-and-conquer merge GEMMs through gemm3 with compact secular vectors

Adds a DC variant of the gemm3 persistent kernel. It reads per-descriptor m/n/k, gathers A rows through a k-index and scatters C columns through a j-index. The secular-equation eigenvectors are now written into a compact, padded U buffer (k_dc_vectors_compact) using per-half slot maps, so the B operand is dense and needs no k-index gather. Large merge levels then use the faster gemm3 path instead of the generic GEMM, and fall back when it declines. This costs a larger U buffer, more index bookkeeping in setup, and added complexity in the kernel's variable-KS pipeline.

```diff
diff --git a/include/springcraft_hip_debug.h b/include/springcraft_hip_debug.h
--- a/include/springcraft_hip_debug.h
+++ b/include/springcraft_hip_debug.h
@@ -15,6 +15,10 @@
 
 int sc_dbg_gemm3_host(sc_ctx* ctx, const double* a, const double* b, double* c, int count, int m, int n, int k, int layout,
                       int lower, double beta);
+
+int sc_dbg_gemm3_dc_host(sc_ctx* ctx, const double* a, const double* b, double* c, int count, int m, int acols, int ccols,
+                         int kmax, int nmax, const int* n, const int* k, const int* a_kidx, const int* c_jidx);
+int sc_dbg_set_gemm3_dc(sc_ctx* ctx, long long min_tiles);
 
 int sc_dbg_symm3_host(sc_ctx* ctx, const double* a, const double* v, double* x, int count, int m, int split);
 int sc_dbg_symm3_stamps(unsigned long long* out4);
diff --git a/springcraft_amd/csrc/api.hip b/springcraft_amd/csrc/api.hip
--- a/springcraft_amd/csrc/api.hip
+++ b/springcraft_amd/csrc/api.hip
@@ -424,6 +424,7 @@
   else if (k == "chase_pair_fallbacks") *value = ctx->cnt_pair_fallbacks;
   else if (k == "xcd_count") *value = ctx->nxcd;
   else if (k == "gemm3_launches") *value = ctx->cnt_gemm3_launches;
+  else if (k == "gemm3_dc_launches") *value = ctx->cnt_gemm3_dc_launches;
   else if (k == "symm3_launches") *value = ctx->cnt_symm3_launches;
   else if (k == "resident_launches") *value = ctx->cnt_resident_launches;
   else if (k == "resident_takeovers") *value = ctx->cnt_resident_takeovers;
diff --git a/springcraft_amd/csrc/common.h b/springcraft_amd/csrc/common.h
--- a/springcraft_amd/csrc/common.h
+++ b/springcraft_amd/csrc/common.h
@@ -55,6 +55,8 @@
   long long cnt_symm3_launches = 0;
   bool gemm3_side_by_side = false;
   long long cnt_gemm3_launches = 0;
+  long long cnt_gemm3_dc_launches = 0;
+  long long gemm3_dc_min_tiles = -1;
   int coop_attr = -1, coop_ok = -1;
   int coop_min_rows = -1;
   int coop_fail_panel = -1;
diff --git a/springcraft_amd/csrc/eigh.hip b/springcraft_amd/csrc/eigh.hip
--- a/springcraft_amd/csrc/eigh.hip
+++ b/springcraft_amd/csrc/eigh.hip
@@ -83,7 +83,7 @@
     P.off_dc = take(dc_slab_doubles(n, &P.DL) * 8 * batch);
     P.off_bt = take(bt_slab_doubles(n, &P.BL) * 8 * batch);
     P.off_qtmp = take((size_t)n * n * 8 * batch);
-    P.off_u = take((size_t)n * n * 8 * batch);
+    P.off_u = take((size_t)dc_u_stride(n) * 8 * batch);
     P.n_merge = 2 * dc_max_nodes(n, P.DL.leaf_max) * batch;
     P.n_bt = bt_desc_count(n, batch);
   }
diff --git a/springcraft_amd/csrc/eigh_internal.h b/springcraft_amd/csrc/eigh_internal.h
--- a/springcraft_amd/csrc/eigh_internal.h
+++ b/springcraft_amd/csrc/eigh_internal.h
@@ -54,6 +54,7 @@
   long long rot_a, rot_b;
   long long ktop_src, ktop_k;
   long long kbot_src, kbot_k;
+  long long slot_top, slot_bot;
   long long cnt;
 };
 
@@ -61,6 +62,7 @@
                   double* d_dc_ws, const DcLayout& DL, double* d_w, long long stride_w,
                   double* d_q_out, double* d_q_tmp, double* d_u, long long stride_q,
                   GemmDesc* d_merge_descs );
+inline long long dc_u_stride(int n) { return (long long)n * ((long long)n + 64); }
 size_t dc_slab_doubles(int n, DcLayout* out);
 int dc_max_nodes(int n, int leaf_max);
 
diff --git a/springcraft_amd/csrc/gemm3.hip b/springcraft_amd/csrc/gemm3.hip
--- a/springcraft_amd/csrc/gemm3.hip
+++ b/springcraft_amd/csrc/gemm3.hip
@@ -32,7 +32,7 @@
   int nwg;
 };
 
-template <int LAYOUT>
+template <int LAYOUT, bool DC = false>
 __global__ __launch_bounds__(1024, 1) void k_gemm3(G3Args P) {
   extern __shared__ __attribute__((aligned(16))) char lds[];
   const int tid = threadIdx.x, lane = tid & 63;
@@ -44,20 +44,36 @@
   const int order = P.order;
   const int nwg = P.nwg;
   const int w_first = order == 0 ? wg : (nwg >> 3) * (wg & 7) + (wg >> 3);
-  struct It { int z, s, r, tm, tn; bool ok; };
-  const int NS = order == 0 ? 1 : (TM + 3) >> 2;
-  auto s_rows = [&](int st) { return order == 0 ? TM : min(4, TM - 4 * st); };
+  struct It { int z, s, r, tm, tn; bool ok; int m, n, ks, tms, tns; };
+  auto tm_of = [&](const It& it) { return DC ? it.tms : TM; };
+  auto tn_of = [&](const It& it) { return DC ? it.tns : TN; };
+  auto ks_of = [&](const It& it) { return DC ? it.ks : KS; };
+  auto m_of = [&](const It& it) { return DC ? it.m : P.m; };
+  auto n_of = [&](const It& it) { return DC ? it.n : P.n; };
+  auto it_load = [&](It& it) {
+    if (DC && it.z < P.count) {
+      const GemmDesc& D = P.descs[it.z];
+      it.m = __builtin_amdgcn_readfirstlane(D.m);
+      it.n = __builtin_amdgcn_readfirstlane(D.n);
+      const int k = __builtin_amdgcn_readfirstlane(D.k);
+      it.ks = max(2, (k + 15) >> 4);
+      it.tms = (it.m + 127) >> 7;
+      it.tns = it.n > 0 ? (it.n + 63) >> 6 : 0;
+    }
+  };
+  auto ns_of = [&](const It& it) { return order == 0 ? 1 : (tm_of(it) + 3) >> 2; };
+  auto s_rows = [&](const It& it, int st) { return order == 0 ? tm_of(it) : min(4, tm_of(it) - 4 * st); };
   auto s_row0 = [&](int st) { return order == 0 ? 0 : 4 * st; };
-  auto s_full = [&](int st) { return lower ? min(TN, 2 * s_row0(st) + 2) : TN; };
-  auto s_len = [&](int st) {
-    const int h = s_rows(st), r0 = s_row0(st), full = s_full(st);
+  auto s_full = [&](const It& it, int st) { return lower ? min(tn_of(it), 2 * s_row0(st) + 2) : tn_of(it); };
+  auto s_len = [&](const It& it, int st) {
+    const int h = s_rows(it, st), r0 = s_row0(st), full = s_full(it, st);
     int len = h * full;
     if (lower)
-      for (int tn = full; tn < TN && (tn >> 1) < r0 + h; ++tn) len += r0 + h - (tn >> 1);
+      for (int tn = full; tn < tn_of(it) && (tn >> 1) < r0 + h; ++tn) len += r0 + h - (tn >> 1);
     return len;
   };
   auto it_decode = [&](It& it) {
-    const int h = s_rows(it.s), r0 = s_row0(it.s), full = s_full(it.s);
+    const int h = s_rows(it, it.s), r0 = s_row0(it.s), full = s_full(it, it.s);
     int r = it.r;
     if (r < h * full) {
       const int c = order == 0 ? r / h : (h == 4 ? r >> 2 : (h == 2 ? r >> 1 : (h == 1 ? r : (r * 43691) >> 17)));
@@ -80,10 +96,10 @@
     it.ok = false;
     for (;;) {
       if (it.z >= P.count) return;
-      const int len = s_len(it.s);
+      const int len = s_len(it, it.s);
       if (it.r < len) break;
       it.r -= len;
-      if (++it.s == NS) { it.s = 0; ++it.z; }
+      if (++it.s >= ns_of(it)) { it.s = 0; ++it.z; it_load(it); }
     }
     it.ok = true;
     it_decode(it);
@@ -91,7 +107,9 @@
   auto it_first = [&]() {
     It it;
     it.z = it.s = it.tm = it.tn = 0;
+    it.m = it.n = it.ks = it.tms = it.tns = 0;
     it.r = w_first;
+    it_load(it);
     it_norm(it);
     return it;
   };
@@ -107,7 +125,15 @@
     const int d = w - 4, q = d & 3, parity = d >> 2;
     It lt = it_first(), cur = lt;
     int l_ks = parity, l_slot = parity % kRing;
-    while (lt.ok && l_ks >= KS) { l_ks -= KS; it_next(lt); }
+    while (lt.ok && l_ks >= ks_of(lt)) { l_ks -= ks_of(lt); it_next(lt); }
+    int kpf = 0;
+    auto prefetch_kidx = [&]() {
+      if (DC && lt.ok) {
+        const int* kix = (const int*)uni64((unsigned long long)(size_t)P.descs[lt.z].a_kidx);
+        kpf = kix[l_ks * 16 + 4 * q + (lane & 3)];
+      }
+    };
+    prefetch_kidx();
     unsigned long long ab_t = 0, bb_t = 0, lda8 = 0, ldb8 = 0;
     unsigned voff_a[4] = {0, 0, 0, 0}, voff_b0 = 0, voff_b1 = 0;
     bool l_new = true;
@@ -115,7 +141,7 @@
       if (l_new) {
         const GemmDesc& D = P.descs[lt.z];
         const int row0 = lt.tm * 128, col0 = lt.tn * 64;
-        const int mrem = min(128, P.m - row0), nrem = min(64, P.n - col0);
+        const int mrem = min(128, m_of(lt) - row0), nrem = min(64, n_of(lt) - col0);
         if (LAYOUT == kGemmAkBk) {
           lda8 = uni64((unsigned long long)D.sa_i * 8ull);
           ab_t = uni64((unsigned long long)(size_t)D.a + (unsigned long long)row0 * lda8);
@@ -143,14 +169,27 @@
       }
       const int k0 = l_ks * 16;
       const int slot_l = l_slot;
+      unsigned kx[4] = {0, 0, 0, 0};
+      if (DC) {
+#pragma unroll
+        for (int i = 0; i < 4; ++i) kx[i] = (unsigned)__builtin_amdgcn_readlane(kpf, i);
+      }
       l_ks += 2;
-      if (l_ks >= KS) { l_ks -= KS; it_next(lt); l_new = true; }
+      if (DC) {
+        while (lt.ok && l_ks >= ks_of(lt)) { l_ks -= ks_of(lt); it_next(lt); l_new = true; }
+        prefetch_kidx();
+      } else if (l_ks >= KS) { l_ks -= KS; it_next(lt); l_new = true; }
       l_slot += 2;
       if (l_slot >= kRing) l_slot -= kRing;
       const unsigned m0v = lds_base + (unsigned)(slot_l * kSlot + q * kQuarter + 2880);
       unsigned long long a0, a1, a2, a3, bb0, bb1;
       if (LAYOUT == kGemmAkBk) {
         a0 = a1 = a2 = a3 = ab_t + (unsigned long long)k0 * 8ull;
+      } else if (DC) {
+        a0 = ab_t + (unsigned long long)kx[0] * lda8;
+        a1 = ab_t + (unsigned long long)kx[1] * lda8;
+        a2 = ab_t + (unsigned long long)kx[2] * lda8;
+        a3 = ab_t + (unsigned long long)kx[3] * lda8;
       } else {
         a0 = ab_t + (unsigned long long)(k0 + 4 * q) * lda8;
         a1 = a0 + lda8; a2 = a1 + lda8; a3 = a2 + lda8;
@@ -188,7 +227,7 @@
         asm volatile("s_waitcnt vmcnt(0)" ::: "memory");
       }
       __builtin_amdgcn_s_barrier();
-      if (++c_ks == KS) { c_ks = 0; it_next(cur); }
+      if (++c_ks == ks_of(cur)) { c_ks = 0; it_next(cur); }
     }
     __builtin_amdgcn_s_barrier();
     return;
@@ -201,17 +240,20 @@
       unsigned long long base, col;
       int row0, colg, mrem, ncol;
       unsigned voff;
+      int jv;
     };
     auto ct_of = [&](const It& it) {
       CT t;
       const GemmDesc& D = P.descs[it.z];
       t.row0 = it.tm * 128;
       t.colg = it.tn * 64 + 16 * cw;
-      t.mrem = min(128, P.m - t.row0);
-      t.ncol = max(0, min(16, P.n - t.colg));
+      t.mrem = min(128, m_of(it) - t.row0);
+      t.ncol = max(0, min(16, n_of(it) - t.colg));
       t.col = uni64((unsigned long long)D.ldc * 8ull);
-      t.base = uni64((unsigned long long)(size_t)D.c + (unsigned long long)t.colg * t.col + (unsigned long long)t.row0 * 8ull);
+      t.base = uni64((unsigned long long)(size_t)D.c + (DC ? 0ull : (unsigned long long)t.colg * t.col) + (unsigned long long)t.row0 * 8ull);
       t.voff = (unsigned)min(lane * 16, (t.mrem - 2) * 8);
+      t.jv = 0;
+      if (DC && lane < t.ncol) t.jv = ((const int*)uni64((unsigned long long)(size_t)D.c_jidx))[t.colg + lane];
       return t;
     };
     auto set_m0 = [&](int h) {
@@ -240,7 +282,7 @@
       const int rel = lower ? max(0, cj - t.row0) : 0;
       if (rel >= t.mrem) return;
       const d2v v = *(const d2v*)(img + j * kRow);
-      const unsigned long long a = t.base + (unsigned long long)j * t.col;
+      const unsigned long long a = t.base + (unsigned long long)(DC ? (unsigned)__builtin_amdgcn_readlane(t.jv, j) : (unsigned)j) * t.col;
       if (rel == 0 && t.mrem == 128) {
         asm volatile("s_nop 4\n\tglobal_store_dwordx4 %0, %1, %2\n\ts_nop 1" : : "v"(voff_st), "v"(v), "s"(a) : "memory");
       } else {
@@ -263,15 +305,25 @@
       set_m0(1);
       for (int j = 8; j < 16; ++j) dma_col(t_cur, j);
     }
+    if (DC && cw == 0) {
+      *(__attribute__((address_space(3))) int*)(lds + kFlagOff) = ks_of(i_cur);
+      asm volatile("s_waitcnt lgkmcnt(0)" ::: "memory");
+    }
     asm volatile("s_waitcnt vmcnt(0)" ::: "memory");
     __builtin_amdgcn_s_barrier();
-    const int cps = KS >= 13 ? 2 : (KS >= 9 ? 4 : 8);
-    const int gsteps = 8 / cps;
-    const int first0 = 1, first1 = 1 + gsteps + (KS >= 9 ? 2 : 1);
+    int cps = KS >= 13 ? 2 : (KS >= 9 ? 4 : 8);
+    int gsteps = 8 / cps;
+    int first0 = 1, first1 = 1 + gsteps + (KS >= 9 ? 2 : 1);
     for (int t = 0; i_cur.ok; ++t) {
       const bool dma_ok = with_c && i_next.ok;
       const bool st_ok = t > 0;
-      for (int ks = 0; ks < KS; ++ks) {
+      const int KSt = ks_of(i_cur);
+      if (DC) {
+        cps = KSt >= 13 ? 2 : (KSt >= 9 ? 4 : (KSt >= 4 ? 8 : 16));
+        gsteps = KSt >= 4 ? 8 / cps : 1;
+        first1 = KSt >= 4 ? 1 + gsteps + (KSt >= 9 ? 2 : 1) : KSt;
+      }
+      for (int ks = 0; ks < KSt; ++ks) {
         int j0 = -1;
         if (ks >= first0 && ks < first0 + gsteps) j0 = (ks - first0) * cps;
         if (ks >= first1 && ks < first1 + gsteps) j0 = 8 + (ks - first1) * cps;
@@ -286,9 +338,9 @@
           }
           asm volatile("s_waitcnt lgkmcnt(0)" ::: "memory");
         }
-        if (dma_ok && ks == KS - 1) asm volatile("s_waitcnt vmcnt(0)" ::: "memory");
-        if (ks == KS - 1 && cw == 0) {
-          *(__attribute__((address_space(3))) int*)(lds + kFlagOff) = i_next.ok ? 1 : 0;
+        if (dma_ok && ks == KSt - 1) asm volatile("s_waitcnt vmcnt(0)" ::: "memory");
+        if (ks == KSt - 1 && cw == 0) {
+          *(__attribute__((address_space(3))) int*)(lds + kFlagOff) = i_next.ok ? (DC ? ks_of(i_next) : 1) : 0;
           asm volatile("s_waitcnt lgkmcnt(0)" ::: "memory");
         }
         __builtin_amdgcn_s_barrier();
@@ -307,6 +359,7 @@
   const int wm = w & 1, wn = w >> 1;
   const int fr = lane & 15, fk = lane >> 4;
   __builtin_amdgcn_s_barrier();
+  int ks_tile = DC ? __builtin_amdgcn_readfirstlane(*(const __attribute__((address_space(3))) int*)(lds + kFlagOff)) : KS;
 
   const unsigned a_base = LAYOUT == kGemmAkBk
                               ? (unsigned)((2 * wm) * kQuarter + (fr >> 3) * kRow + (((fk >> 1) * 8 + (fr & 7)) * 16) + (fk & 1) * 8)
@@ -406,7 +459,7 @@
                  : "memory");
     __builtin_amdgcn_s_barrier();
     const char* sn = lds + slot * kSlot;
-    const bool boundary = ks == KS - 1;
+    const bool boundary = ks == ks_tile - 1;
     ks = boundary ? 0 : ks + 1;
     read_frags_asm(2, lds_base + (unsigned)(slot * kSlot));
     __builtin_amdgcn_sched_barrier(0);
@@ -416,7 +469,9 @@
     read_frags(1, sn, 1);
     if (boundary) {
       swap_all();
-      more = __builtin_amdgcn_readfirstlane(*(const __attribute__((address_space(3))) int*)(lds + kFlagOff)) != 0;
+      const int flag = __builtin_amdgcn_readfirstlane(*(const __attribute__((address_space(3))) int*)(lds + kFlagOff));
+      more = flag != 0;
+      if (DC) ks_tile = flag;
     }
     mfmas(2);
   }
@@ -451,19 +506,23 @@
   return total <= 0x3fffffffLL;
 }
 
+namespace {
+bool gemm3_lds_ok(sc_ctx* ctx) {
+  if (ctx->gemm3_attr < 0) {
+    bool ok = true;
+    for (const void* f : {reinterpret_cast<const void*>(&k_gemm3<kGemmAmBk>), reinterpret_cast<const void*>(&k_gemm3<kGemmAkBk>),
+                          reinterpret_cast<const void*>(&k_gemm3<kGemmAmBn>), reinterpret_cast<const void*>(&k_gemm3<kGemmAmBk, true>)})
+      ok = hipFuncSetAttribute(f, hipFuncAttributeMaxDynamicSharedMemorySize, kG3Lds) == hipSuccess && ok;
+    ctx->gemm3_attr = ok ? 1 : 0;
+  }
+  return ctx->gemm3_attr == 1;
+}
+}
+
 int launch_gemm3_uniform(sc_ctx* ctx, const GemmDesc* d_desc, int count, int m, int n, int k, int layout, int lower,
                          double alpha, double beta, bool aligned16) {
   if (!gemm3_would_take(ctx, count, m, n, k, layout, lower, alpha, beta, aligned16)) return 1;
-  if (ctx->gemm3_attr < 0) {
-    const bool ok0 = hipFuncSetAttribute(reinterpret_cast<const void*>(&k_gemm3<kGemmAmBk>),
-                                         hipFuncAttributeMaxDynamicSharedMemorySize, kG3Lds) == hipSuccess &&
-                     hipFuncSetAttribute(reinterpret_cast<const void*>(&k_gemm3<kGemmAkBk>),
-                                         hipFuncAttributeMaxDynamicSharedMemorySize, kG3Lds) == hipSuccess;
-    const bool ok2 = hipFuncSetAttribute(reinterpret_cast<const void*>(&k_gemm3<kGemmAmBn>),
-                                         hipFuncAttributeMaxDynamicSharedMemorySize, kG3Lds) == hipSuccess;
-    ctx->gemm3_attr = (ok0 && ok2) ? 1 : 0;
-  }
-  if (ctx->gemm3_attr != 1) return 1;
+  if (!gemm3_lds_ok(ctx)) return 1;
   static const int env_order = [] { const char* e = getenv("SPRINGCRAFT_GEMM3_ORDER"); return e ? atoi(e) : 1; }();
   static const int env_lower_wgs = [] { const char* e = getenv("SPRINGCRAFT_GEMM3_LOWER_WGS"); return e ? std::max(8, std::min(256, atoi(e) / 8 * 8)) : 0; }();
   const int nwg = lower ? (env_lower_wgs > 0 ? env_lower_wgs : (ctx->gemm3_side_by_side ? 224 : 256)) : 256;
@@ -477,6 +536,100 @@
     return 1;
   }
   ++ctx->cnt_gemm3_launches;
+  return SC_OK;
+}
+
+bool gemm3_dc_would_take(const sc_ctx* ctx, int count, int max_m, int max_n) {
+  static const int env = [] { const char* e = getenv("SPRINGCRAFT_GEMM3"); return e ? atoi(e) : 1; }();
+  const char* e_dc = getenv("SPRINGCRAFT_GEMM3_DC");
+  if (env == 0 || (e_dc && atoi(e_dc) == 0) || count <= 0 || max_m < 2 || max_n < 1) return false;
+  if (ctx->num_cus < 256 || ctx->gemm3_attr == 0) return false;
+  const long long total = (long long)count * ((max_m + 127) / 128) * ((max_n + 63) / 64);
+  const long long dbg = ctx->gemm3_dc_min_tiles;
+  const long long need = dbg >= 0 ? dbg : (env == 2 || dbg == -2 ? 0 : 4LL * 256);
+  static const int env_rows = [] { const char* e = getenv("SPRINGCRAFT_GEMM3_DC_ROWS"); return e ? atoi(e) : 512; }();
+  if (dbg == -1 && env != 2 && max_m < env_rows) return false;
+  return total >= need && total <= 0x3fffffffLL;
+}
+
+int launch_gemm3_dc(sc_ctx* ctx, const GemmDesc* d_desc, int count, int max_m, int max_n) {
+  if (!gemm3_dc_would_take(ctx, count, max_m, max_n)) return 1;
+  if (ctx->gemm3_dc_min_tiles == -2) return 1;
+  if (!gemm3_lds_ok(ctx)) return 1;
+  static const int env_order = [] { const char* e = getenv("SPRINGCRAFT_GEMM3_ORDER"); return e ? atoi(e) : 1; }();
+  G3Args A{d_desc, count, 0, 0, 0, 0, 0, g_gemm3_order >= 0 ? g_gemm3_order : env_order, 256};
+  hipLaunchKernelGGL((k_gemm3<kGemmAmBk, true>), dim3(256), dim3(1024), kG3Lds, ctx->stream, A);
+  if (hipGetLastError() != hipSuccess) {
+    ctx->gemm3_attr = 0;
+    return 1;
+  }
+  ++ctx->cnt_gemm3_launches;
+  ++ctx->cnt_gemm3_dc_launches;
+  return SC_OK;
+}
+
+extern "C" int sc_dbg_gemm3_dc_host(sc_ctx* ctx, const double* a, const double* b, double* c, int count, int m, int acols,
+                                    int ccols, int kmax, int nmax, const int* n, const int* k, const int* a_kidx,
+                                    const int* c_jidx) {
+  if (!ctx || !a || !b || !c || !n || !k || !a_kidx || !c_jidx || count < 1 || m < 2 || (m & 1) || acols < 1 || ccols < 1 ||
+      kmax < 1 || nmax < 1)
+    return SC_ERR_INVALID_ARG;
+  for (int z = 0; z < count; ++z) {
+    if (n[z] < 0 || n[z] > nmax || k[z] < 0 || k[z] > kmax) return SC_ERR_INVALID_ARG;
+    for (int i = 0; i < k[z]; ++i)
+      if (a_kidx[(size_t)z * kmax + i] < 0 || a_kidx[(size_t)z * kmax + i] >= acols) return SC_ERR_INVALID_ARG;
+    for (int j = 0; j < n[z]; ++j)
+      if (c_jidx[(size_t)z * nmax + j] < 0 || c_jidx[(size_t)z * nmax + j] >= ccols) return SC_ERR_INVALID_ARG;
+  }
+  SC_HIP(ctx, hipSetDevice(ctx->device));
+  const int kp = 16 * std::max(2, (kmax + 15) / 16);
+  const size_t ea = (size_t)m * acols, eb = (size_t)kp * nmax, ec = (size_t)m * ccols;
+  const size_t ints = ((size_t)kp + nmax + 3) / 4 * 4;
+  char* base = nullptr;
+  SC_HIP(ctx, hipMalloc((void**)&base, (ea + eb + ec) * count * 8 + ints * 4 * count + sizeof(GemmDesc) * (size_t)count + 256));
+  double* da = (double*)base;
+  double* db = da + ea * count;
+  double* dc = db + eb * count;
+  int* di = (int*)(dc + ec * count);
+  GemmDesc* dd = (GemmDesc*)(di + ints * count);
+  std::vector<double> hb(eb * count, 0.0);
+  std::vector<int> hi(ints * count, 0);
+  std::vector<GemmDesc> h((size_t)count);
+  for (int z = 0; z < count; ++z) {
+    for (int j = 0; j < nmax; ++j)
+      for (int i = 0; i < k[z]; ++i) hb[eb * z + (size_t)j * kp + i] = b[((size_t)z * nmax + j) * kmax + i];
+    for (int i = 0; i < k[z]; ++i) hi[ints * z + i] = a_kidx[(size_t)z * kmax + i];
+    for (int j = 0; j < n[z]; ++j) hi[ints * z + kp + j] = c_jidx[(size_t)z * nmax + j];
+    GemmDesc D{};
+    D.a = da + ea * z; D.b = db + eb * z; D.c = dc + ec * z;
+    D.m = m; D.n = n[z]; D.k = k[z]; D.ldc = m; D.alpha = 1.0; D.beta = 0.0;
+    D.sa_i = 1; D.sa_k = m; D.sb_k = 1; D.sb_j = kp;
+    D.a_kidx = di + ints * z; D.c_jidx = di + ints * z + kp;
+    h[(size_t)z] = D;
+  }
+  int rc = SC_OK;
+  auto fail = [&](hipError_t e) { if (e != hipSuccess && rc == SC_OK) rc = sc_set_error(ctx, SC_ERR_HIP, "%s", hipGetErrorString(e)); };
+  fail(hipMemcpy(da, a, ea * count * 8, hipMemcpyHostToDevice));
+  fail(hipMemcpy(db, hb.data(), eb * count * 8, hipMemcpyHostToDevice));
+  fail(hipMemcpy(dc, c, ec * count * 8, hipMemcpyHostToDevice));
+  fail(hipMemcpy(di, hi.data(), ints * 4 * count, hipMemcpyHostToDevice));
+  fail(hipMemcpy(dd, h.data(), sizeof(GemmDesc) * (size_t)count, hipMemcpyHostToDevice));
+  if (rc == SC_OK) {
+    const long long keep = ctx->gemm3_dc_min_tiles;
+    ctx->gemm3_dc_min_tiles = 0;
+    const int took = launch_gemm3_dc(ctx, dd, count, m, nmax);
+    ctx->gemm3_dc_min_tiles = keep;
+    if (took != SC_OK) rc = sc_set_error(ctx, SC_ERR_INVALID_ARG, "k_gemm3 is not available on this device");
+    fail(hipStreamSynchronize(ctx->stream));
+  }
+  if (rc == SC_OK) fail(hipMemcpy(c, dc, ec * count * 8, hipMemcpyDeviceToHost));
+  (void)hipFree(base);
+  return rc;
+}
+
+extern "C" int sc_dbg_set_gemm3_dc(sc_ctx* ctx, long long min_tiles) {
+  if (!ctx) return SC_ERR_INVALID_ARG;
+  ctx->gemm3_dc_min_tiles = min_tiles;
   return SC_OK;
 }
 
diff --git a/springcraft_amd/csrc/gemm_f64.h b/springcraft_amd/csrc/gemm_f64.h
--- a/springcraft_amd/csrc/gemm_f64.h
+++ b/springcraft_amd/csrc/gemm_f64.h
@@ -35,5 +35,8 @@
 bool gemm3_would_take(sc_ctx* ctx, int count, int m, int n, int k, int layout, int lower, double alpha, double beta,
                       bool aligned16);
 
+int launch_gemm3_dc(sc_ctx* ctx, const GemmDesc* d_desc, int count, int max_m, int max_n);
+bool gemm3_dc_would_take(const sc_ctx* ctx, int count, int max_m, int max_n);
+
 int launch_symm3(sc_ctx* ctx, const GemmDesc* d_desc, int count, int m, int split, bool aligned16, bool any_size = false);
 bool symm3_would_take(sc_ctx* ctx, int count, int m, int split, bool aligned16);
diff --git a/springcraft_amd/csrc/stedc.hip b/springcraft_amd/csrc/stedc.hip
--- a/springcraft_amd/csrc/stedc.hip
+++ b/springcraft_amd/csrc/stedc.hip
@@ -1,4 +1,5 @@
 #include <algorithm>
+#include <cstdlib>
 #include <vector>
 
 #include "eigh_internal.h"
@@ -11,6 +12,8 @@
 __device__ __forceinline__ const int* iptr(const double* ws, long long off) {
   return reinterpret_cast<const int*>(ws + off);
 }
+
+__host__ __device__ __forceinline__ int dc_kpad(int k) { return 16 * (k > 16 ? (k + 15) / 16 : 2); }
 
 __device__ __forceinline__ double wave_sum_all(double v) {
 #pragma unroll
@@ -183,7 +186,8 @@
                                                    const double* __restrict__ q_all, long long stride_q,
                                                    long long w_old_off, GemmDesc* __restrict__ descs,
                                                    int use_lds, double* __restrict__ gscratch,
-                                                   long long gscratch_stride) {
+                                                   long long gscratch_stride, double* __restrict__ u_all,
+                                                   long long stride_u, int compact) {
   extern __shared__ __attribute__((aligned(16))) double lds[];
   __shared__ double red[16];
   __shared__ double s_tol;
@@ -272,6 +276,8 @@
   int* ktop_k = iptr(ws, DL.ktop_k);
   int* kbot_src = iptr(ws, DL.kbot_src);
   int* kbot_k = iptr(ws, DL.kbot_k);
+  int* slot_top = iptr(ws, DL.slot_top);
+  int* slot_bot = iptr(ws, DL.slot_bot);
   __shared__ int wsum[3][16];
   __shared__ int s_nrot;
   const int L = (N + nthr - 1) / nthr;
@@ -384,8 +390,9 @@
         ws[DL.zz + lo + K] = sz[j];
         src[lo + K] = scol[j];
         const bool top = scol[j] < mid;
-        if (top || smix[j]) { ktop_src[lo + K1] = scol[j]; ktop_k[lo + K1] = K; ++K1; }
-        if (!top || smix[j]) { kbot_src[lo + K3] = scol[j]; kbot_k[lo + K3] = K; ++K3; }
+        slot_top[lo + K] = slot_bot[lo + K] = -1;
+        if (top || smix[j]) { ktop_src[lo + K1] = scol[j]; ktop_k[lo + K1] = K; slot_top[lo + K] = K1; ++K1; }
+        if (!top || smix[j]) { kbot_src[lo + K3] = scol[j]; kbot_k[lo + K3] = K; slot_bot[lo + K] = K3; ++K3; }
         ++K;
       }
     }
@@ -398,6 +405,17 @@
       GemmDesc& Db = descs[((size_t)b * nodes_in_level + g) * 2 + 1];
       Db.n = ts;
       Db.k = tb;
+      if (compact) {
+        double* ub = u_all + (size_t)b * stride_u + (size_t)lo * n;
+        Dt.b = ub;
+        Dt.sb_j = dc_kpad(tt);
+        Db.b = ub + (size_t)dc_kpad(tt) * ts;
+        Db.sb_j = dc_kpad(tb);
+      }
+    }
+    if (compact) {
+      for (int i = tt + tid; i < dc_kpad(tt); i += nthr) ktop_src[lo + i] = lo;
+      for (int i = tb + tid; i < dc_kpad(tb); i += nthr) kbot_src[lo + i] = lo;
     }
   }
 }
@@ -657,6 +675,65 @@
   for (int i = threadIdx.x; i < K; i += blockDim.x) U[i] *= inv;
 }
 
+constexpr int kVecCap = 24;
+__global__ __launch_bounds__(256) void k_dc_vectors_compact(double* __restrict__ dc_all, DcLayout DL,
+                                                            const DcNode* __restrict__ nodes, int nodes_in_level,
+                                                            const GemmDesc* __restrict__ descs,
+                                                            double* __restrict__ u_all, long long stride_u) {
+  __shared__ double red[4];
+  const int g = blockIdx.y, b = blockIdx.z;
+  const DcNode nd = nodes[g];
+  double* ws = dc_all + (size_t)b * DL.slab;
+  const int K = iptr(ws, DL.cnt)[2 * g];
+  const int j = blockIdx.x;
+  if (j >= K) return;
+  const int lo = nd.lo, n = DL.n, tid = threadIdx.x;
+  const int tt = descs[((size_t)b * nodes_in_level + g) * 2].k, tb = descs[((size_t)b * nodes_in_level + g) * 2 + 1].k;
+  const int ldt = dc_kpad(tt), ldb = dc_kpad(tb);
+  const double* dl = ws + DL.dl + lo;
+  const double* zh = ws + DL.zhat + lo;
+  const int* st = iptr(ws, DL.slot_top) + lo;
+  const int* sb = iptr(ws, DL.slot_bot) + lo;
+  const double dorg = dl[iptr(ws, DL.org)[lo + j]];
+  const double tau = ws[DL.tauv + lo + j];
+  double* ub = u_all + (size_t)b * stride_u + (size_t)lo * n;
+  double* UT = ub + (size_t)j * ldt;
+  double* UB = ub + (size_t)ldt * K + (size_t)j * ldb;
+  double uv[kVecCap];
+  double ss = 0.0;
+#pragma unroll
+  for (int t = 0; t < kVecCap; ++t) {
+    const int i = tid + 256 * t;
+    uv[t] = 0.0;
+    if (i < K) {
+      uv[t] = zh[i] / ((dl[i] - dorg) - tau);
+      ss += uv[t] * uv[t];
+    }
+  }
+  for (int i = tid + 256 * kVecCap; i < K; i += 256) {
+    const double u = zh[i] / ((dl[i] - dorg) - tau);
+    ss += u * u;
+  }
+  ss = wave_sum_all(ss);
+  if ((tid & 63) == 0) red[tid >> 6] = ss;
+  __syncthreads();
+  const double inv = 1.0 / sqrt((red[0] + red[1]) + (red[2] + red[3]));
+  auto put = [&](int i, double u) {
+    const double v = u * inv;
+    const int s1 = st[i], s2 = sb[i];
+    if (s1 >= 0) UT[s1] = v;
+    if (s2 >= 0) UB[s2] = v;
+  };
+#pragma unroll
+  for (int t = 0; t < kVecCap; ++t) {
+    const int i = tid + 256 * t;
+    if (i < K) put(i, uv[t]);
+  }
+  for (int i = tid + 256 * kVecCap; i < K; i += 256) put(i, zh[i] / ((dl[i] - dorg) - tau));
+  for (int i = tt + tid; i < ldt; i += 256) UT[i] = 0.0;
+  for (int i = tb + tid; i < ldb; i += 256) UB[i] = 0.0;
+}
+
 __global__ __launch_bounds__(256) void k_dc_finalize(double* __restrict__ dc_all, DcLayout DL,
                                                      const DcNode* __restrict__ nodes, long long w_new_off) {
   const int g = blockIdx.y, b = blockIdx.z;
@@ -743,6 +820,19 @@
   return t;
 }
 
+bool dc_level_compact(const sc_ctx* ctx, const std::vector<DcNode>& nodes, int n, int batch, long long stride_q,
+                      long long stride_u, int* max_m_out) {
+  int max_m = 0, max_n = 0;
+  bool even = n >= 256 && !(n & 1) && !(stride_q & 1) && !(stride_u & 1);
+  for (const DcNode& nd : nodes) {
+    if (((nd.lo | nd.mid | nd.hi) & 1) || nd.hi - nd.lo < 128) even = false;
+    max_m = std::max(max_m, std::max(nd.mid - nd.lo, nd.hi - nd.mid));
+    max_n = std::max(max_n, nd.hi - nd.lo);
+  }
+  *max_m_out = max_m;
+  return even && gemm3_dc_would_take(ctx, 2 * (int)nodes.size() * batch, max_m, max_n);
+}
+
 constexpr int kLeafMax = 32;
 constexpr int kLdsCapSetup = 7000;
 constexpr int kLdsCapSecular = 9800;
@@ -768,6 +858,7 @@
   L.zhat = take(nn); L.rot_c = take(nn); L.rot_s = take(nn); L.scale = take(8);
   L.src = take(nn); L.org = take(nn); L.dest = take(nn); L.rot_a = take(nn); L.rot_b = take(nn);
   L.ktop_src = take(nn); L.ktop_k = take(nn); L.kbot_src = take(nn); L.kbot_k = take(nn);
+  L.slot_top = take(nn); L.slot_bot = take(nn);
   L.cnt = take(2LL * dc_max_nodes(n, kLeafMax) + 8);
   L.slab = off;
   if (out) *out = L;
@@ -813,9 +904,13 @@
 
   auto qbuf = [&](int stage) { return ((nlev - stage) % 2 == 0) ? d_q_out : d_q_tmp; };
 
+  const long long stride_u = dc_u_stride(n);
   std::vector<GemmDesc> h_descs;
   std::vector<size_t> desc_off(nlev);
+  std::vector<char> compact(nlev);
+  std::vector<int> max_m(nlev);
   for (int l = 0; l < nlev; ++l) {
+    compact[l] = dc_level_compact(ctx, tree.levels[l], n, batch, stride_q, stride_u, &max_m[l]) ? 1 : 0;
     desc_off[l] = h_descs.size();
     const auto& nodes = tree.levels[l];
     const double* q_old = qbuf(l);
@@ -830,9 +925,9 @@
           D.a = q_old + (size_t)b * stride_q + r0;
           D.sa_i = 1; D.sa_k = n;
           D.a_kidx = ip(half == 0 ? DL.ktop_src : DL.kbot_src);
-          D.b = d_u + (size_t)b * stride_q + (size_t)nd.lo * n + nd.lo;
+          D.b = d_u + (size_t)b * stride_u + (size_t)nd.lo * n + nd.lo;
           D.sb_k = 1; D.sb_j = n;
-          D.b_kidx = ip(half == 0 ? DL.ktop_k : DL.kbot_k);
+          D.b_kidx = compact[l] ? nullptr : ip(half == 0 ? DL.ktop_k : DL.kbot_k);
           D.c = q_new + (size_t)b * stride_q + r0;
           D.ldc = n;
           D.c_jidx = ip(DL.dest);
@@ -871,7 +966,8 @@
       const size_t lds = use_lds ? (size_t)maxN * 22 + 32 : 0;
       const int threads = maxN >= 1024 ? 1024 : (maxN >= 256 ? 256 : 64);
       hipLaunchKernelGGL(k_dc_setup, dim3((unsigned)G, (unsigned)batch), dim3(threads), lds, st, d_dc_ws, DL,
-                         dn, G, q_old, stride_q, w_old, descs, use_lds, d_big, (long long)3 * n);
+                         dn, G, q_old, stride_q, w_old, descs, use_lds, d_big, (long long)3 * n, d_u, stride_u,
+                         (int)compact[l]);
     }
     hipLaunchKernelGGL(k_dc_rotate, dim3((unsigned)((maxN + 255) / 256), (unsigned)G, (unsigned)batch),
                        dim3(256), 0, st, d_dc_ws, DL, dn, q_old, stride_q);
@@ -885,15 +981,20 @@
     }
     hipLaunchKernelGGL(k_dc_zhat, dim3((unsigned)((maxN + 3) / 4), (unsigned)G, (unsigned)batch), dim3(256), 0,
                        st, d_dc_ws, DL, dn);
-    hipLaunchKernelGGL(k_dc_vectors, dim3((unsigned)maxN, (unsigned)G, (unsigned)batch), dim3(256), 0, st,
-                       d_dc_ws, DL, dn, d_u, stride_q);
+    if (compact[l])
+      hipLaunchKernelGGL(k_dc_vectors_compact, dim3((unsigned)maxN, (unsigned)G, (unsigned)batch), dim3(256), 0, st,
+                         d_dc_ws, DL, dn, G, descs, d_u, stride_u);
+    else
+      hipLaunchKernelGGL(k_dc_vectors, dim3((unsigned)maxN, (unsigned)G, (unsigned)batch), dim3(256), 0, st,
+                         d_dc_ws, DL, dn, d_u, stride_u);
     hipLaunchKernelGGL(k_dc_finalize, dim3((unsigned)((maxN + 255) / 256), (unsigned)G, (unsigned)batch),
                        dim3(256), 0, st, d_dc_ws, DL, dn, w_new);
     hipLaunchKernelGGL(k_dc_copy_deflated, dim3((unsigned)maxN, (unsigned)G, (unsigned)batch), dim3(256), 0, st,
                        d_dc_ws, DL, dn, q_old, q_new, stride_q);
     t_gemm.start();
-    SC_TRY(launch_gemm_f64(ctx, descs, 2 * G * batch, (maxN + 1) / 2, maxN, kGemmTile, 1, true, false,
-                           kGemmAmBk));
+    if (!compact[l] || launch_gemm3_dc(ctx, descs, 2 * G * batch, max_m[l], maxN) != SC_OK)
+      SC_TRY(launch_gemm_f64(ctx, descs, 2 * G * batch, max_m[l], maxN, kGemmTile, 1, true, false,
+                             kGemmAmBk));
     t_gemm.stop();
   }
   const long long w_final = (nlev % 2 == 0) ? DL.w0 : DL.w1;
```

New measurement: 181,300 modes/s, median of 6. 1.2% higher.
